# johannes-graeter/limo

Hardware: NVIDIA H100
Metric: BA windows/s (30 KF, 3k LM, 40k obs) (higher is better)
Workload: dtype f64

## Files before the change

limo_b200/csrc/kba_api.cu:

```cuda
#include <algorithm>
#include <atomic>
#include <chrono>
#include <cstdio>
#include <cstdlib>
#include <cstring>
#include <memory>
#include <string>
#include <thread>
#include <vector>

#include <cuda_runtime.h>

#include "kba_b200.h"
#include "kba_kernels.h"

using namespace kba;

static thread_local std::string g_last_error;
static thread_local bool g_force_host_pack = false;
static int fail(int code, const std::string& msg) {
    g_last_error = msg;
    return code;
}
#define CU(call)                                                                                              \
// ... 9 lines not shown
    bool own_stream = false;
    Counters counters;
    bool kernel_timing = false;
    cudaEvent_t ev0 = nullptr, ev1 = nullptr;
    std::vector<cudaEvent_t> ev_pool;
    int ev_used = 0;
    int sm_count = 132;
    cudaEvent_t ev_block = nullptr;
    bool blocking_sync = false;
    void* ws = nullptr;
    size_t ws_cap = 0;
};

static cudaError_t wait_event(kba_handle*, cudaEvent_t ev) { return cudaEventSynchronize(ev); }
static cudaError_t wait_stream(kba_handle* h) {
    if (!h->blocking_sync) return cudaStreamSynchronize(h->stream);
    if (!h->ev_block) {
        const cudaError_t e = cudaEventCreateWithFlags(&h->ev_block, cudaEventBlockingSync | cudaEventDisableTiming);
        if (e != cudaSuccess) return e;
    }
    const cudaError_t e = cudaEventRecord(h->ev_block, h->stream);
    if (e != cudaSuccess) return e;
    return cudaEventSynchronize(h->ev_block);
}

template <typename T>
struct Staged {
    T* h = nullptr;
    T* d = nullptr;
    size_t n = 0;
    int alloc(size_t count, bool host_copy) {
        n = count;
        const size_t bytes = std::max<size_t>(count, 1) * sizeof(T);
        if (cudaMalloc(&d, bytes) != cudaSuccess) return 1;
        if (host_copy && cudaMallocHost(&h, bytes) != cudaSuccess) return 1;
        return 0;
    }
    void release() {
        if (d) cudaFree(d);
        if (h) cudaFreeHost(h);
        d = nullptr; h = nullptr;
    }
    cudaError_t upload(cudaStream_t s) { return cudaMemcpyAsync(d, h, std::max<size_t>(n, 1) * sizeof(T), cudaMemcpyHostToDevice, s); }
    cudaError_t download(cudaStream_t s) { return cudaMemcpyAsync(h, d, std::max<size_t>(n, 1) * sizeof(T), cudaMemcpyDeviceToHost, s); }
};

struct kba_batch {
    kba_handle* h = nullptr;
    BatchDev bd{};
    std::vector<WinDesc> desc_h;
    Staged<WinDesc> desc;
    Staged<double> pose0, plane0, cam, lm0, lm_weight;
    Staged<uint8_t> kf_fixed;
    Staged<int> lm_ptr, obs_kf, obs_cam, obs_lm, kf_ptr, pm_lm, pm_cam, chunk_lm0, chunk_lm1, chunk_k0, chunk_k1, lm_orig, obs_orig;
    Staged<int> grp_k0, grp_k1;
    bool device_pack = false;
    Staged<int> r_lm_ptr, r_obs_kf, r_obs_cam, r_gp_lm;
    Staged<float> r_obs_u, r_obs_v, r_obs_d;
    Staged<double> r_lm_pos, r_lm_weight;
    Staged<double> lm_user;
    Staged<uint8_t> rej_user;
    PackRaw raw;
    Staged<int> obs_rank;
    Staged<float> obs_u, obs_v, obs_d, pm_u, pm_v, pm_d;
    Staged<WinState> state;
    Staged<IterRecord> log;
    Staged<double> pose_out[2], lm_out[2], plane_out[2];
    Staged<int> gp_lm, gp_kf, gp_of_lm, gp_shared;
    Staged<double> gp_weight;
    Staged<uint8_t> lm_active;
    Staged<int> n_active;
    Staged<unsigned long long> jac_obs;
    std::vector<void*> scratch;
    LaunchCfg lc;
    size_t h2d_bytes = 0, d2h_bytes = 0;
    float last_solve_ms = 0.f;
    cudaEvent_t ev_a = nullptr, ev_b = nullptr, ev_poll = nullptr, ev_poll2 = nullptr;
    struct SolveGraph {
        cudaGraph_t graph = nullptr;
        cudaGraphExec_t exec = nullptr;
        std::vector<unsigned char> key;
        Counters per_pass;
        int mode = 0, passes_per_launch = 0;
        bool unusable = false;
        void destroy() {
            if (exec) cudaGraphExecDestroy(exec);
            if (graph) cudaGraphDestroy(graph);
            exec = nullptr; graph = nullptr; key.clear();
        }
    } sg;
    Staged<int> loop_pass;
    long long solves_done = 0;
    int p_split_cap = 0;

    template <typename T>
    int dev_alloc(T** p, size_t count) {
        void* q = nullptr;
        if (cudaMalloc(&q, std::max<size_t>(count, 1) * sizeof(T)) != cudaSuccess) return 1;
        scratch.push_back(q);
        *p = (T*)q;
        return 0;
    }
    void dev_free(void* q) {
        scratch.erase(std::remove(scratch.begin(), scratch.end(), q), scratch.end());
        cudaFree(q);
    }
    void release() {
        desc.release(); pose0.release(); plane0.release(); cam.release(); lm0.release(); lm_weight.release();
        kf_fixed.release(); lm_ptr.release(); obs_kf.release(); obs_cam.release(); obs_lm.release(); kf_ptr.release();
        pm_lm.release(); pm_cam.release(); chunk_lm0.release(); chunk_lm1.release(); chunk_k0.release(); chunk_k1.release();
        lm_orig.release(); obs_orig.release(); obs_rank.release(); obs_u.release(); obs_v.release();
        grp_k0.release(); grp_k1.release();
        r_lm_ptr.release(); r_obs_kf.release(); r_obs_cam.release(); r_gp_lm.release(); r_obs_u.release(); r_obs_v.release();
        r_obs_d.release(); r_lm_pos.release(); r_lm_weight.release(); lm_user.release(); rej_user.release();
        obs_d.release(); pm_u.release(); pm_v.release(); pm_d.release(); state.release(); log.release();
        pose_out[0].release(); pose_out[1].release(); lm_out[0].release(); lm_out[1].release(); lm_active.release();
        n_active.release(); jac_obs.release(); plane_out[0].release(); plane_out[1].release();
        gp_lm.release(); gp_kf.release(); gp_of_lm.release(); gp_weight.release(); gp_shared.release();
        for (void* p : scratch) cudaFree(p);
        scratch.clear();
        if (ev_a) cudaEventDestroy(ev_a);
        if (ev_b) cudaEventDestroy(ev_b);
        if (ev_poll) cudaEventDestroy(ev_poll);
        if (ev_poll2) cudaEventDestroy(ev_poll2);
        sg.destroy();
        loop_pass.release();
    }
};

struct MotionBufs {
    Staged<unsigned char> up;
    Staged<unsigned char> out;
    double* run_pw = nullptr, *trim_val = nullptr;
    unsigned char* run_active = nullptr, *run_rej = nullptr;
    IterRecord* log = nullptr;
    cudaEvent_t ev0 = nullptr, ev1 = nullptr;
    int frames_cap = 0, runs_cap = 0, meas_cap = 0;
    std::vector<unsigned> seen;
    unsigned stamp = 0;
    static size_t al(size_t b) { return (b + 15) & ~(size_t)15; }
    static size_t up_bytes(int frames, int runs, int meas) {
        return al(sizeof(FrameDesc) * (size_t)frames) + al(4 * ((size_t)runs + frames)) + 5 * al(4 * (size_t)meas);
    }
    static size_t out_bytes(int frames, int log_cap, int runs) {
        return al(sizeof(FrameRes) * (size_t)frames) + al(sizeof(IterRecord) * (size_t)frames * log_cap) + al((size_t)runs);
    }
    int alloc(int frames, int runs, int meas) {
        frames_cap = frames; runs_cap = runs; meas_cap = meas;
        int bad = up.alloc(up_bytes(frames, runs, meas), true) | out.alloc(out_bytes(frames, kIterLogCap, runs), true);
        bad |= cudaMalloc(&run_pw, sizeof(double) * 4 * (size_t)std::max(runs, 1)) != cudaSuccess;
        bad |= cudaMalloc(&trim_val, sizeof(double) * 2 * (size_t)std::max(runs, 1)) != cudaSuccess;
        bad |= cudaMalloc(&run_active, (size_t)std::max(runs, 1)) != cudaSuccess;
        bad |= cudaMalloc(&run_rej, (size_t)std::max(runs, 1)) != cudaSuccess;
        bad |= cudaMalloc(&log, sizeof(IterRecord) * kIterLogCap * (size_t)frames) != cudaSuccess;
        bad |= cudaEventCreate(&ev0) != cudaSuccess;
        bad |= cudaEventCreate(&ev1) != cudaSuccess;
        return bad;
    }
    ~MotionBufs() {
        up.release(); out.release();
        if (run_pw) cudaFree(run_pw);
        if (trim_val) cudaFree(trim_val);
        if (run_active) cudaFree(run_active);
        if (run_rej) cudaFree(run_rej);
        if (log) cudaFree(log);
        if (ev0) cudaEventDestroy(ev0);
        if (ev1) cudaEventDestroy(ev1);
    }
};

struct TrackSolver {
// ... 186 lines not shown
            const int k = b->obs_kf.h[(size_t)d.obs_off + o];
            k0 = std::min(k0, k); k1 = std::max(k1, k);
        }
        for (int j = j0; j < j1; ++j)
            if (gp_kf_of_lm[j] >= 0) { k0 = std::min(k0, gp_kf_of_lm[j]); k1 = std::max(k1, gp_kf_of_lm[j]); }
        b->grp_k0.h[d.grp_off + c] = k0;
        b->grp_k1.h[d.grp_off + c] = k1;
    }
}

static void fill_window_raw(kba_batch* b, int wi, const kba_window* w) {
    const WinDesc& d = b->desc_h[wi];
    memcpy(b->pose0.h + 7 * (size_t)d.kf_off, w->kf_pose, sizeof(double) * 7 * w->n_kf);
    memcpy(b->kf_fixed.h + d.kf_off, w->kf_fixed, w->n_kf);
    for (int k = 0; k < w->n_kf; ++k) {
        double* pl = b->plane0.h + 4 * (size_t)(d.kf_off + k);
        if (w->kf_plane) memcpy(pl, w->kf_plane + 4 * k, 4 * sizeof(double));
        else { pl[0] = 0; pl[1] = 0; pl[2] = 1; pl[3] = 0; }
    }
    for (int c = 0; c < w->n_cam; ++c) {
        double* o = b->cam.h + kCamStride * (size_t)(d.cam_off + c);
        quat_to_rot<double>(w->cam_pose + 7 * c, o);
        o[9] = w->cam_pose[7 * c + 4]; o[10] = w->cam_pose[7 * c + 5]; o[11] = w->cam_pose[7 * c + 6];
        o[12] = w->cam_intr[3 * c]; o[13] = w->cam_intr[3 * c + 1]; o[14] = w->cam_intr[3 * c + 2]; o[15] = 0;
    }
    const size_t nl = (size_t)w->n_lm, no = (size_t)w->n_obs;
    memcpy(b->r_lm_pos.h + 3 * (size_t)d.lm_off, w->lm_pos, 3 * nl * sizeof(double));
    memcpy(b->r_lm_weight.h + d.lm_off, w->lm_weight, nl * sizeof(double));
    int* lp = b->r_lm_ptr.h + d.lm_off + wi;
    if (nl) memcpy(lp, w->lm_obs_ptr, (nl + 1) * sizeof(int)); else lp[0] = 0;
    memcpy(b->r_obs_kf.h + d.obs_off, w->obs_kf, no * sizeof(int));
    if (w->obs_cam) memcpy(b->r_obs_cam.h + d.obs_off, w->obs_cam, no * sizeof(int));
    else memset(b->r_obs_cam.h + d.obs_off, 0, no * sizeof(int));
    memcpy(b->r_obs_u.h + d.obs_off, w->obs_u, no * sizeof(float));
    memcpy(b->r_obs_v.h + d.obs_off, w->obs_v, no * sizeof(float));
    memcpy(b->r_obs_d.h + d.obs_off, w->obs_d, no * sizeof(float));
    if (w->n_gp) {
        memcpy(b->r_gp_lm.h + d.gp_off, w->gp_lm, w->n_gp * sizeof(int));
        memcpy(b->gp_kf.h + d.gp_off, w->gp_kf, w->n_gp * sizeof(int));
        memcpy(b->gp_weight.h + d.gp_off, w->gp_weight, w->n_gp * sizeof(double));
    }
    int max_rank = 0;
    for (int j = 0; j < w->n_lm; ++j) {
        int rank = 0;
        for (int o = w->lm_obs_ptr[j] + 1; o < w->lm_obs_ptr[j + 1]; ++o) {
            rank = (w->obs_kf[o] == w->obs_kf[o - 1]) ? rank + 1 : 0;
            max_rank = std::max(max_rank, rank);
        }
    }
    b->desc_h[wi].max_rank = max_rank;
    b->desc.h[wi].max_rank = max_rank;
}

static int window_rows(const kba_window& w) {
    const bool planes = w.n_gp > 0 || w.plane_reg_weight > 0;
    int n_free = 0;
    for (int k = 0; k < w.n_kf; ++k) n_free += w.kf_fixed[k] ? 0 : 1;
    return (planes ? 10 : 6) * n_free + 1;
}

struct kba_shard_comm;
kba::Exchange kba_shard_exchange(kba_shard_comm* c);

static int solve_graph_mode() {
    static const int m = [] {
        const char* e = getenv("KBA_GRAPH");
        const int v = e ? atoi(e) : 2;
        return (v < 0 || v > 2) ? 2 : v;
    }();
    return m;
}

static bool shard_graph_enabled() {
    static const bool on = [] { const char* e = getenv("KBA_SHARD_GRAPH"); return e ? atoi(e) != 0 : true; }();
    return on;
}

template <typename T>
static void key_append(std::vector<unsigned char>& k, const T& v) {
    const unsigned char* p = reinterpret_cast<const unsigned char*>(&v);
    k.insert(k.end(), p, p + sizeof(T));
}

static bool build_solve_graph(kba_batch* b, const SolveParams& sp, const LaunchCfg& lc, int mode, int max_passes, int check_every,
                              const std::vector<unsigned char>& key) {
    kba_batch::SolveGraph& g = b->sg;
    g.destroy();
    cudaStream_t s = b->h->stream;
    Counters per{};
    cudaError_t e = cudaSuccess;
    bool capturing = false;
    int rc_pass = 0;
    if (mode == 2) {
        cudaGraphConditionalHandle handle = 0;
        cudaGraphNode_t node = nullptr;
        cudaGraphNodeParams np = {};
        e = cudaGraphCreate(&g.graph, 0);
        if (e == cudaSuccess) e = cudaGraphConditionalHandleCreate(&handle, g.graph, 1, cudaGraphCondAssignDefault);
        if (e == cudaSuccess) {
            np.type = cudaGraphNodeTypeConditional;
            np.conditional.handle = handle;
            np.conditional.type = cudaGraphCondTypeWhile;
            np.conditional.size = 1;
            e = cudaGraphAddNode(&node, g.graph, nullptr, 0, &np);
        }
        if (e == cudaSuccess) e = cudaStreamBeginCaptureToGraph(s, np.conditional.phGraph_out[0], nullptr, nullptr, 0, cudaStreamCaptureModeThreadLocal);
        if (e == cudaSuccess) {
            capturing = true;
            rc_pass = launch_pass(b->bd, sp, lc, &per, s);
            launch_loop_cond(b->bd, (unsigned long long)handle, b->loop_pass.d, max_passes, s);
            cudaGraph_t body = nullptr;
            e = cudaStreamEndCapture(s, &body);
            capturing = false;
        }
        g.passes_per_launch = 0;
    } else {
        e = cudaStreamBeginCapture(s, cudaStreamCaptureModeThreadLocal);
        if (e == cudaSuccess) {
            capturing = true;
            for (int i = 0; i < check_every && !rc_pass; ++i) rc_pass = launch_pass(b->bd, sp, lc, i == 0 ? &per : nullptr, s);
            launch_count_active(b->bd, s);
            b->n_active.download(s);
            e = cudaStreamEndCapture(s, &g.graph);
            capturing = false;
        }
        g.passes_per_launch = check_every;
    }
    if (capturing) { cudaGraph_t junk = nullptr; cudaStreamEndCapture(s, &junk); }
    if (e == cudaSuccess && rc_pass) e = cudaErrorUnknown;
    if (e == cudaSuccess) e = cudaGraphInstantiate(&g.exec, g.graph, 0);
    if (e != cudaSuccess) {
        if (getenv("KBA_GRAPH_VERBOSE")) fprintf(stderr, "kba: solve graph (mode %d) not available: %s -- stream launches\n", mode, cudaGetErrorString(e));
        g.destroy();
        g.unusable = true;
        cudaGetLastError();
        return false;
    }
    if (getenv("KBA_GRAPH_VERBOSE")) fprintf(stderr, "kba: solve graph built (mode %d, %lld launches per pass)\n", mode, per.launches_total);
    g.key = key;
    g.per_pass = per;
    g.mode = mode;
    return true;
}

static void add_pass_counters(Counters& c, const Counters& per, long long passes) {
    c.launches_total += per.launches_total * passes; c.launches_jacobian += per.launches_jacobian * passes;
    c.launches_prep += per.launches_prep * passes; c.launches_schur += per.launches_schur * passes;
    c.launches_solve += per.launches_solve * passes; c.launches_backsub += per.launches_backsub * passes;
    c.launches_cost += per.launches_cost * passes; c.launches_update += per.launches_update * passes;
    c.launches_trim += per.launches_trim * passes;
}

extern "C" {

int kba_version(void) { return KBA_VERSION_MAJOR * 100 + KBA_VERSION_MINOR; }
int kba_internal_stream(kba_handle* h, cudaStream_t* s, int* device) {
    if (!h) return fail(KBA_ERR_BAD_ARG, "null handle");
    *s = h->stream; *device = h->device;
    return KBA_OK;
}
int kba_internal_fail(int code, const char* msg) { return fail(code, msg ? msg : ""); }
int kba_internal_workspace(kba_handle* h, size_t bytes, void** out) {
    if (!h || !out) return fail(KBA_ERR_BAD_ARG, "null handle");
    if (bytes > h->ws_cap) {
        CU(cudaSetDevice(h->device));
        CU(cudaStreamSynchronize(h->stream));
        if (h->ws) cudaFree(h->ws);
        h->ws = nullptr; h->ws_cap = 0;
        const size_t cap = bytes + bytes / 4 + 4096;
        CU(cudaMalloc(&h->ws, cap));
        h->ws_cap = cap;
    }
    *out = h->ws;
    return KBA_OK;
}
const char* kba_last_error(void) { return g_last_error.c_str(); }

void kba_default_options(kba_options* o) {
    if (!o) return;
    memset(o, 0, sizeof *o);
    o->depth_thres = 0.16; o->reprojection_thres = 1.6;
    o->depth_quantile = 0.95; o->reprojection_quantile = 0.95; o->gp_quantile = 1.0; o->gp_huber = 0.1;
    o->num_trim_rounds = -1; o->trim_solver_iterations = 2; o->final_solver_iterations = 100;
    o->min_landmarks_for_trimming = 100; o->min_residual_groups = 30; o->num_rounds_option = 1;
    o->solver_time_sec = 20.0;
    o->function_tolerance = 1e-6; o->gradient_tolerance = 1e-10; o->parameter_tolerance = 1e-8;
    o->initial_trust_region_radius = 1e4; o->max_trust_region_radius = 1e16; o->min_trust_region_radius = 1e-32;
    o->min_relative_decrease = 1e-3; o->min_lm_diagonal = 1e-6; o->max_lm_diagonal = 1e32;
    o->max_consecutive_invalid_steps = 5; o->precision = 0;
}

int kba_create(kba_handle** out, int device) {
    if (!out) return fail(KBA_ERR_BAD_ARG, "null out pointer");
    int n = 0;
    if (cudaGetDeviceCount(&n) != cudaSuccess || n == 0)
        return fail(KBA_ERR_CUDA, "no CUDA device available: the kba_b200 library has no CPU fallback");
    if (device < 0 || device >= n) return fail(KBA_ERR_BAD_ARG, "device index out of range");
    CU(cudaSetDevice(device));
    cudaDeviceProp prop;
    CU(cudaGetDeviceProperties(&prop, device));
    if (prop.major != 9 || prop.minor != 0)
        return fail(KBA_ERR_CUDA, "kba_b200 kernels are built for sm_90a (H100) only, device " + std::to_string(device) +
                                      " is sm_" + std::to_string(prop.major) + std::to_string(prop.minor));
    kba_handle* h = new kba_handle();
    h->device = device;
    h->sm_count = prop.multiProcessorCount;
    { const char* e = std::getenv("KBA_BLOCKING_SYNC"); h->blocking_sync = e && std::atoi(e) != 0; }
    CU(cudaStreamCreateWithFlags(&h->stream, cudaStreamNonBlocking));
    h->own_stream = true;
    CU(cudaEventCreate(&h->ev0));
    CU(cudaEventCreate(&h->ev1));
    *out = h;
    return KBA_OK;
}

void kba_destroy(kba_handle* h) {
    if (!h) return;
    if (h->own_stream && h->stream) cudaStreamDestroy(h->stream);
    if (h->ev0) cudaEventDestroy(h->ev0);
    if (h->ev1) cudaEventDestroy(h->ev1);
    if (h->ev_block) cudaEventDestroy(h->ev_block);
// ... 31 lines not shown

static int syrk_split(int nr_cap_max, int n_windows, int sm_count) {
    const int nb = nr_cap_max / 64, pairs = nb * (nb + 1) / 2;
    return std::min(16, (6 * sm_count + n_windows * pairs - 1) / (n_windows * pairs));
}

static void solve_layout(BatchDev& bd, int nr_cap_max, int n_windows, int sm_count) {
    bd.solve_tiled = (nr_cap_max <= 192 && !bd.solve_row_major) ? 1 : 0;
    const int split_dflt = (!bd.solve_tiled && n_windows <= 16) ? std::max(1, std::min(32, sm_count / n_windows)) : 0;
    const char* e = std::getenv("KBA_SOLVE_SPLIT");
    bd.solve_split = bd.solve_tiled ? 0 : (e ? std::atoi(e) : split_dflt);
}

static int batch_create(kba_handle* h, int32_t n_windows, const kba_window* w, const int* rows_of, bool track_large, kba_batch** out) {
    if (!h || !w || !out || n_windows <= 0) return fail(KBA_ERR_BAD_ARG, "bad argument to kba_batch_create");
    CU(cudaSetDevice(h->device));
    std::string why;
    for (int i = 0; i < n_windows; ++i) {
        const int rc = validate_window(&w[i], why);
        if (rc != KBA_OK) return fail(rc, "window " + std::to_string(i) + ": " + why);
        if (w[i].n_kf < 3 && !w[i].landmarks_fixed)
            return fail(KBA_ERR_NOT_ENOUGH_KF, "window " + std::to_string(i) + ": fewer than 3 keyframes");
    }
    kba_batch* b = new kba_batch();
    b->h = h;
    BatchDev& bd = b->bd;
    bd.n_win = n_windows;
    b->desc_h.resize(n_windows);
    long long kf = 0, cam = 0, lm = 0, obs = 0, chunks = 0, soff = 0, gp = 0, groups = 0;
    int max_rows = 0, max_rows_free = 0, max_groups = 1;
    int nr_cap_max = 64;
    for (int i = 0; i < n_windows; ++i) {
        WinDesc& d = b->desc_h[i];
        memset(&d, 0, sizeof d);
        d.n_kf = w[i].n_kf; d.n_cam = w[i].n_cam; d.n_lm = w[i].n_lm; d.n_obs = w[i].n_obs; d.n_gp = w[i].n_gp;
        d.kf_off = (int)kf; d.cam_off = (int)cam; d.lm_off = (int)lm; d.obs_off = (int)obs; d.gp_off = (int)gp;
        d.chunk_off = (int)chunks; d.n_chunks = (w[i].n_lm + 31) / 32;
        d.grp_off = (int)groups; d.n_groups = (w[i].n_lm + 7) / 8;
        groups += d.n_groups; max_groups = std::max(max_groups, d.n_groups);
        max_rows_free = std::max(max_rows_free, window_rows(w[i]));
        d.scale_kf0 = w[i].scale_kf0; d.scale_kf1 = w[i].scale_kf1;
        d.scale_weight = w[i].scale_weight; d.scale_value = w[i].scale_value;
        const bool planes = w[i].n_gp > 0 || w[i].plane_reg_weight > 0;
        const int rows = rows_of ? rows_of[i] : (planes ? 10 : 6) * w[i].n_kf + 1;
        max_rows = std::max(max_rows, rows);
        d.nr_cap = ((rows + 63) / 64) * 64;
        d.plane_reg_weight = w[i].plane_reg_weight; d.plane_dist_fixed = w[i].plane_dist_fixed;
        d.s_off = soff;
        soff += (long long)d.nr_cap * d.nr_cap;
        nr_cap_max = std::max(nr_cap_max, d.nr_cap);
        kf += w[i].n_kf; cam += w[i].n_cam; lm += w[i].n_lm; obs += w[i].n_obs; chunks += d.n_chunks; gp += w[i].n_gp;
        bd.max_obs = std::max(bd.max_obs, w[i].n_obs); bd.max_lm = std::max(bd.max_lm, w[i].n_lm);
        bd.max_kf = std::max(bd.max_kf, w[i].n_kf); bd.max_gp = std::max(bd.max_gp, w[i].n_gp);
    }
    if (obs > 2000000000LL) { b->release(); delete b; return fail(KBA_ERR_CAPACITY, "batch exceeds 2^31 observations"); }
    if (nr_cap_max > 640) {
        b->release();
        delete b;
        return fail(KBA_ERR_CAPACITY, "reduced system larger than 640 rows (106 keyframes, or 63 with ground-plane blocks)");
    }
    bd.tot_kf = kf; bd.tot_cam = cam; bd.tot_lm = lm; bd.tot_obs = obs; bd.tot_chunks = (int)chunks; bd.tot_gp = gp;
    bd.tot_groups = (int)groups;
    bd.nr_cap_max = nr_cap_max;
    b->lc.nr_cap_max = nr_cap_max;
    b->lc.sm_count = h->sm_count;
    {
        int max_chunks = 1;
        for (auto& d : b->desc_h) max_chunks = std::max(max_chunks, d.n_chunks);
        int p = syrk_split(nr_cap_max, n_windows, h->sm_count);
        b->lc.small_syrk = (max_rows <= 184);
        if (b->lc.small_syrk) p = (h->sm_count + n_windows - 1) / n_windows;
        bd.p_split = std::max(1, std::min(p, max_chunks));
        const char* fe = std::getenv("KBA_FUSED");
        bd.fused = (b->lc.small_syrk && bd.max_kf <= kFusedMaxKf && !(fe && std::atoi(fe) == 0)) ? 1 : 0;
        if (const char* pe = std::getenv("KBA_P_SPLIT")) { if (std::atoi(pe) > 0) p = std::atoi(pe); }
        if (bd.fused) bd.p_split = std::max(1, std::min(p, max_groups));
        else if (std::getenv("KBA_P_SPLIT")) bd.p_split = std::max(1, std::min(p, max_chunks));
        b->lc.fused_slots = (max_rows_free <= 176) ? 6 : 7;
    }
    bd.cost_parts = std::max((bd.max_obs + 255) / 256, (bd.max_obs / 16 + bd.max_lm / 32 + 4 + 7) / 8);
    { const char* le = std::getenv("KBA_LINEARIZE"); b->lc.lin_fused = !(le && std::atoi(le) == 0); }
    { const char* le = std::getenv("KBA_LIN_GRID"); if (le) b->lc.lin_grid = std::max(-1, std::atoi(le)); }
    { const char* le = std::getenv("KBA_BS_GRID"); if (le) b->lc.bs_grid = std::max(-1, std::atoi(le)); }
    {
        auto knob = [](const char* name, int dflt) { const char* e = std::getenv(name); return e ? std::atoi(e) : dflt; };
        bd.eval_tiles_jac = std::max(1, knob("KBA_EVAL_TILES_JAC", 8));
        bd.eval_tiles_cost = std::max(1, knob("KBA_EVAL_TILES_COST", 8));
        bd.eval_min_blocks = knob("KBA_EVAL_MIN_BLOCKS", 2);
        bd.eval_cs = knob("KBA_EVAL_CS", 0);
        bd.solve_row_major = knob("KBA_SOLVE_ROW_MAJOR", 0);
        solve_layout(bd, nr_cap_max, n_windows, h->sm_count);
    }
    bd.bs_parts = (bd.max_lm + 15) / 16;
    {
        const char* pe = std::getenv("KBA_DEVICE_PACK");
        b->device_pack = (bd.fused || track_large) && !g_force_host_pack && bd.max_lm <= pack_max_landmarks() && !(pe && std::atoi(pe) == 0);
    }
    if (track_large) {
        int max_chunks = 1;
        for (auto& d : b->desc_h) max_chunks = std::max(max_chunks, d.n_chunks);
        int p = syrk_split(192, n_windows, h->sm_count);
        if (const char* pe = std::getenv("KBA_P_SPLIT")) { if (std::atoi(pe) > 0) p = std::atoi(pe); }
        bd.p_split = std::max(bd.p_split, std::max(1, std::min(p, max_chunks)));
        b->p_split_cap = bd.p_split;
    }
    const bool hp = !b->device_pack;
    int bad = 0;
    bad |= b->desc.alloc(n_windows, true);
    bad |= b->pose0.alloc(7 * kf, true); bad |= b->plane0.alloc(4 * kf, true); bad |= b->kf_fixed.alloc(kf, true);
    bad |= b->cam.alloc(kCamStride * cam, true);
    bad |= b->lm0.alloc(3 * lm, hp); bad |= b->lm_weight.alloc(lm, hp); bad |= b->lm_ptr.alloc(lm + n_windows, hp);
    bad |= b->obs_kf.alloc(obs, hp); bad |= b->obs_cam.alloc(obs, hp); bad |= b->obs_lm.alloc(obs, hp);
    bad |= b->obs_u.alloc(obs, hp); bad |= b->obs_v.alloc(obs, hp); bad |= b->obs_d.alloc(obs, hp);
    bad |= b->kf_ptr.alloc(kf + n_windows, hp); bad |= b->pm_lm.alloc(obs, hp); bad |= b->pm_cam.alloc(obs, hp);
    bad |= b->pm_u.alloc(obs, hp); bad |= b->pm_v.alloc(obs, hp); bad |= b->pm_d.alloc(obs, hp);
    bad |= b->chunk_lm0.alloc(chunks, hp); bad |= b->chunk_lm1.alloc(chunks, hp);
    bad |= b->chunk_k0.alloc(chunks, hp); bad |= b->chunk_k1.alloc(chunks, hp);
    bad |= b->lm_orig.alloc(lm, hp); bad |= b->obs_rank.alloc(obs, hp);
    if (hp) bad |= b->obs_orig.alloc(obs, true);
    bad |= b->grp_k0.alloc(groups, hp); bad |= b->grp_k1.alloc(groups, hp);
    if (b->device_pack) {
        bad |= b->r_lm_ptr.alloc(lm + n_windows, true); bad |= b->r_obs_kf.alloc(obs, true); bad |= b->r_obs_cam.alloc(obs, true);
        bad |= b->r_obs_u.alloc(obs, true); bad |= b->r_obs_v.alloc(obs, true); bad |= b->r_obs_d.alloc(obs, true);
        bad |= b->r_lm_pos.alloc(3 * lm, true); bad |= b->r_lm_weight.alloc(lm, true); bad |= b->r_gp_lm.alloc(gp, true);
        bad |= b->lm_user.alloc(3 * lm, true); bad |= b->rej_user.alloc(lm, true);
        bad |= b->dev_alloc(&b->raw.lm_inv, lm);
    }
    bad |= b->dev_alloc(&bd.grp_t0, groups); bad |= b->dev_alloc(&bd.grp_t1, groups); bad |= b->dev_alloc(&bd.grp_rs, groups);
    bad |= b->dev_alloc(&bd.grp_tiles, groups);
    bad |= b->dev_alloc(&bd.lin_tile, (size_t)(obs / 16) + (size_t)(lm / 32) + 4 * (size_t)n_windows + 4);
#ifdef KBA_PROF
    bad |= b->dev_alloc(&bd.prof, 16);
    if (!bad) cudaMemset(bd.prof, 0, 16 * sizeof(unsigned long long));
#endif
    bad |= b->dev_alloc(&bd.rt[0], (size_t)kPoseStride * kf); bad |= b->dev_alloc(&bd.rt[1], (size_t)kPoseStride * kf);
    {
        bd.panel_cap = 0;
        bd.vpanel = nullptr;
        bad |= b->dev_alloc(&bd.chunk_poff, chunks); bad |= b->dev_alloc(&bd.chunk_rs, chunks);
    }
    bad |= b->dev_alloc(&bd.chunk_t0, chunks); bad |= b->dev_alloc(&bd.chunk_t1, chunks); bad |= b->dev_alloc(&bd.obs_row, obs);
    bad |= b->state.alloc(n_windows, true); bad |= b->log.alloc((size_t)n_windows * kIterLogCap, true);
    for (int q = 0; q < 2; ++q) { bad |= b->pose_out[q].alloc(7 * kf, true); bad |= b->lm_out[q].alloc(3 * lm, hp); }
    bad |= b->lm_active.alloc(lm, hp); bad |= b->n_active.alloc(1, true); bad |= b->jac_obs.alloc(1, true);
    bad |= b->plane_out[0].alloc(4 * kf, true); bad |= b->plane_out[1].alloc(4 * kf, true);
    bad |= b->gp_lm.alloc(gp, hp); bad |= b->gp_kf.alloc(gp, true); bad |= b->gp_weight.alloc(gp, true); bad |= b->gp_of_lm.alloc(lm, hp); bad |= b->gp_shared.alloc(gp, hp);
    bad |= b->dev_alloc(&bd.gp_lin, 14 * gp); bad |= b->dev_alloc(&bd.vgp, 30 * gp);
    bad |= b->dev_alloc(&bd.gp_cost_x, n_windows); bad |= b->dev_alloc(&bd.gp_cost_c, n_windows);
    bad |= b->dev_alloc(&bd.off_pose, kf); bad |= b->dev_alloc(&bd.off_dir, kf); bad |= b->dev_alloc(&bd.off_dist, kf);
    bad |= b->dev_alloc(&bd.bkf, 27 * kf);
    bad |= b->dev_alloc(&bd.scale_f, (size_t)n_windows * nr_cap_max); bad |= b->dev_alloc(&bd.lambda_f, (size_t)n_windows * nr_cap_max);
    bad |= b->dev_alloc(&bd.grad_f, (size_t)n_windows * nr_cap_max); bad |= b->dev_alloc(&bd.delta_f, (size_t)n_windows * nr_cap_max);
    bad |= b->dev_alloc(&bd.lm_scale, 3 * lm); bad |= b->dev_alloc(&bd.lm_linv, 6 * lm); bad |= b->dev_alloc(&bd.lm_z, 3 * lm);
    bad |= b->dev_alloc(&bd.lm_g, 3 * lm); bad |= b->dev_alloc(&bd.lm_lambda, 3 * lm); bad |= b->dev_alloc(&bd.trim_val, 3 * lm);
    bad |= b->dev_alloc(&bd.trim_reject, lm);
    bad |= b->dev_alloc(&bd.res, 3 * obs); bad |= b->dev_alloc(&bd.jp, 18 * obs);
    if (!bd.fused) bad |= b->dev_alloc(&bd.jl, 9 * obs);
    else { bad |= b->dev_alloc(&bd.vobs, 18 * obs); bad |= b->dev_alloc(&bd.lm_run, lm); }
    bad |= b->dev_alloc(&bd.cost_part_x, (size_t)n_windows * bd.cost_parts); bad |= b->dev_alloc(&bd.cost_part_c, (size_t)n_windows * bd.cost_parts);
    bad |= b->dev_alloc(&bd.bs_part, (size_t)n_windows * bd.bs_parts * 4);
    bad |= b->dev_alloc(&bd.sred, (size_t)soff * bd.p_split); bad |= b->dev_alloc(&bd.amat, (size_t)soff);
    bad |= b->dev_alloc(&bd.chol_w, (size_t)n_windows * 32 * 32); bad |= b->dev_alloc(&bd.chol_invd, (size_t)n_windows * nr_cap_max);
    if (bad) {
        const std::string msg = std::string("device/pinned allocation failed: ") + cudaGetErrorString(cudaGetLastError());
        b->release(); delete b;
        return fail(KBA_ERR_CUDA, msg);
// ... 114 lines not shown
        for (int i = 0; i < n_windows; ++i) { b->desc_h[i].panel_off = (long long)i * b->bd.panel_cap; b->desc.h[i].panel_off = b->desc_h[i].panel_off; }
    }
    cudaStream_t s = b->h->stream;
    if (b->device_pack) {
        CU(b->desc.upload(s)); CU(b->pose0.upload(s)); CU(b->plane0.upload(s)); CU(b->kf_fixed.upload(s)); CU(b->cam.upload(s));
        CU(b->r_lm_pos.upload(s)); CU(b->r_lm_weight.upload(s)); CU(b->r_lm_ptr.upload(s));
        CU(b->r_obs_kf.upload(s)); CU(b->r_obs_cam.upload(s)); CU(b->r_obs_u.upload(s)); CU(b->r_obs_v.upload(s)); CU(b->r_obs_d.upload(s));
        CU(b->r_gp_lm.upload(s)); CU(b->gp_kf.upload(s)); CU(b->gp_weight.upload(s));
        launch_pack(b->bd, b->raw, s);
        CU(cudaGetLastError());
        const BatchDev& bd = b->bd;
        b->h2d_bytes = sizeof(WinDesc) * bd.n_win + (7 + 4) * 8 * bd.tot_kf + bd.tot_kf + kCamStride * 8 * bd.tot_cam +
                       (3 + 1) * 8 * bd.tot_lm + 4 * (bd.tot_lm + bd.n_win) + (2 * 4 + 3 * 4) * bd.tot_obs + (4 + 4 + 8) * bd.tot_gp;
        return KBA_OK;
    }
    CU(b->desc.upload(s)); CU(b->pose0.upload(s)); CU(b->plane0.upload(s)); CU(b->kf_fixed.upload(s)); CU(b->cam.upload(s));
    CU(b->lm0.upload(s)); CU(b->lm_weight.upload(s)); CU(b->lm_ptr.upload(s));
    CU(b->obs_kf.upload(s)); CU(b->obs_cam.upload(s)); CU(b->obs_lm.upload(s));
    CU(b->obs_u.upload(s)); CU(b->obs_v.upload(s)); CU(b->obs_d.upload(s));
    CU(b->kf_ptr.upload(s)); CU(b->pm_lm.upload(s)); CU(b->pm_cam.upload(s)); CU(b->pm_u.upload(s)); CU(b->pm_v.upload(s)); CU(b->pm_d.upload(s));
    CU(b->chunk_lm0.upload(s)); CU(b->chunk_lm1.upload(s)); CU(b->chunk_k0.upload(s)); CU(b->chunk_k1.upload(s));
    CU(b->grp_k0.upload(s)); CU(b->grp_k1.upload(s));
    CU(b->lm_orig.upload(s)); CU(b->obs_rank.upload(s));
    CU(b->gp_lm.upload(s)); CU(b->gp_kf.upload(s)); CU(b->gp_weight.upload(s)); CU(b->gp_of_lm.upload(s)); CU(b->gp_shared.upload(s));
    const BatchDev& bd = b->bd;
    b->h2d_bytes = sizeof(WinDesc) * bd.n_win + (7 + 4) * 8 * bd.tot_kf + bd.tot_kf + kCamStride * 8 * bd.tot_cam +
                   (3 + 1) * 8 * bd.tot_lm + 4 * (bd.tot_lm + bd.n_win) + (3 * 4 + 3 * 4) * bd.tot_obs +
                   4 * (bd.tot_kf + bd.n_win) + (2 * 4 + 3 * 4) * bd.tot_obs + 8 * bd.tot_chunks + 8 * bd.tot_groups;
    return KBA_OK;
}

static SolveParams make_params(const kba_options* o) {
    SolveParams sp;
    sp.gp_huber = o->gp_huber; sp.gp_quantile = o->gp_quantile;
    sp.depth_thres = o->depth_thres; sp.reprojection_thres = o->reprojection_thres;
    sp.depth_quantile = o->depth_quantile; sp.reprojection_quantile = o->reprojection_quantile;
    sp.function_tolerance = o->function_tolerance; sp.gradient_tolerance = o->gradient_tolerance;
    sp.parameter_tolerance = o->parameter_tolerance; sp.initial_radius = o->initial_trust_region_radius;
    sp.max_radius = o->max_trust_region_radius; sp.min_radius = o->min_trust_region_radius;
    sp.min_relative_decrease = o->min_relative_decrease; sp.min_lm_diagonal = o->min_lm_diagonal;
    sp.max_lm_diagonal = o->max_lm_diagonal; sp.trim_solver_iterations = o->trim_solver_iterations;
    sp.final_solver_iterations = o->final_solver_iterations; sp.min_residual_groups = o->min_residual_groups;
    sp.max_consecutive_invalid_steps = o->max_consecutive_invalid_steps;
    sp.max_solver_time = o->solver_time_sec;
    return sp;
}

int kba_batch_solve(kba_batch* b, const kba_options* opt) {
    if (!b || !opt) return fail(KBA_ERR_BAD_ARG, "bad argument to kba_batch_solve");
    if (opt->precision != 0 && opt->precision != 1) return fail(KBA_ERR_BAD_ARG, "kba_options.precision must be 0 (FP64) or 1 (FP32 linearisation)");
    if (opt->num_trim_rounds > 6 || (opt->num_trim_rounds < 0 && opt->num_rounds_option > 6))
        return fail(KBA_ERR_CAPACITY, "at most 6 trimming rounds (KBA_MAX_SOLVES = 8 inner solves incl. one retry and the final solve)");
    b->bd.precision = opt->precision;
    b->bd.lin1 = (b->bd.fused && b->lc.lin_fused && opt->precision == 0 && b->lc.max_rank == 0) ? 1 : 0;
    kba_handle* h = b->h;
    CU(cudaSetDevice(h->device));
    cudaStream_t s = h->stream;
    const SolveParams sp = make_params(opt);
    LaunchCfg lc = b->lc;
    lc.rounds_override = opt->num_trim_rounds;
    lc.min_landmarks_for_trimming = opt->min_landmarks_for_trimming;
    lc.num_rounds_option = opt->num_rounds_option;
    lc.time_jacobian = h->kernel_timing;
    if (h->kernel_timing && h->ev_pool.empty()) {
        h->ev_pool.resize(1024);
        for (auto& e : h->ev_pool) CU(cudaEventCreate(&e));
    }
    h->ev_used = 0;
    lc.ev_pool = h->ev_pool.data(); lc.ev_cap = (int)h->ev_pool.size(); lc.ev_used = &h->ev_used;
    CU(cudaMemsetAsync(b->bd.jac_obs, 0, sizeof(unsigned long long), s));
    CU(cudaMemsetAsync(b->bd.cost_part_x, 0, sizeof(double) * (size_t)b->bd.n_win * b->bd.cost_parts, s));
    CU(cudaMemsetAsync(b->bd.cost_part_c, 0, sizeof(double) * (size_t)b->bd.n_win * b->bd.cost_parts, s));
    CU(cudaEventRecord(b->ev_a, s));
    launch_reset(b->bd, lc, s);
    const int rounds_max = 7;
    const int max_passes = rounds_max * (3 * opt->trim_solver_iterations + 4) + opt->final_solver_iterations + 8;
    const auto t0 = std::chrono::steady_clock::now();
    int check_every = 4;
    bool timed_out = false, poll_pending = false;
    int gmode = solve_graph_mode();
    if (h->kernel_timing || launch_check_enabled() || s == nullptr || b->sg.unusable) gmode = 0;
    const bool lockstep = b->bd.sharded != 0;
    if (lockstep) gmode = (gmode && shard_graph_enabled() && b->solves_done > 0) ? 1 : 0;
    if (gmode) {
        std::vector<unsigned char> key;
        key.reserve(sizeof(BatchDev) + sizeof(SolveParams) + 64);
        key_append(key, b->bd); key_append(key, sp); key_append(key, gmode); key_append(key, max_passes); key_append(key, s);
        key_append(key, lc.nr_cap_max); key_append(key, lc.max_rank); key_append(key, (int)lc.small_syrk); key_append(key, (int)lc.lin_fused);
        key_append(key, lc.fused_slots); key_append(key, lc.xchg.user);
        key_append(key, lc.lin_grid); key_append(key, lc.bs_grid);
        if (!(b->sg.exec && b->sg.key == key) && !build_solve_graph(b, sp, lc, gmode, max_passes, check_every, key)) gmode = 0;
    }
    if (gmode == 2) {
        CU(cudaMemsetAsync(b->loop_pass.d, 0, sizeof(int), s));
        CU(cudaGraphLaunch(b->sg.exec, s));
        CU(b->loop_pass.download(s));
        CU(cudaEventRecord(b->ev_b, s));
        CU(b->jac_obs.download(s));
        CU(wait_stream(h));
        CU(cudaGetLastError());
        CU(cudaEventElapsedTime(&b->last_solve_ms, b->ev_a, b->ev_b));
        h->counters.jacobian_obs += (long long)b->jac_obs.h[0];
        add_pass_counters(h->counters, b->sg.per_pass, b->loop_pass.h[0]);
        h->counters.launches_total += b->loop_pass.h[0];
        b->solves_done++;
        return KBA_OK;
    }
    if (gmode == 1) {
        cudaEvent_t evs[2] = {b->ev_poll, b->ev_poll2};
        const int n_launch = (max_passes + check_every - 1) / check_every;
        int launched = 0;
        for (int g = 0; g < n_launch; ++g) {
            CU(cudaGraphLaunch(b->sg.exec, s));
            ++launched;
            CU(cudaEventRecord(evs[g & 1], s));
            if (lockstep) {
                CU(wait_event(h, evs[g & 1]));
                if (b->n_active.h[0] == 0) break;
            } else if (g >= 1) {
                CU(wait_event(h, evs[(g - 1) & 1]));
                if (b->n_active.h[0] == 0) break;
                if (opt->solver_time_sec > 0) {
                    const double el = std::chrono::duration<double>(std::chrono::steady_clock::now() - t0).count();
                    if (el > KBA_MAX_SOLVES * opt->solver_time_sec + 2.0) { timed_out = true; break; }
                }
            }
        }
        if (timed_out) g_last_error = "kba_batch_solve: host safety cap reached, unfinished windows carry KBA_ERR_TIMEOUT in kba_result.status";
        CU(cudaEventRecord(b->ev_b, s));
        CU(b->jac_obs.download(s));
        CU(wait_stream(h));
        CU(cudaGetLastError());
        CU(cudaEventElapsedTime(&b->last_solve_ms, b->ev_a, b->ev_b));
        h->counters.jacobian_obs += (long long)b->jac_obs.h[0];
        add_pass_counters(h->counters, b->sg.per_pass, (long long)launched * check_every);
        h->counters.launches_total += launched;
        b->solves_done++;
        return KBA_OK;
    }
    for (int pass = 0; pass < max_passes; ++pass) {
        if (launch_pass(b->bd, sp, lc, &h->counters, s)) {
            cudaEventRecord(b->ev_b, s);
            return KBA_ERR_NCCL;
        }
        if (pass < 2) {
            const cudaError_t le = cudaGetLastError();
            if (le != cudaSuccess) { cudaEventRecord(b->ev_b, s); cudaStreamSynchronize(s); return fail(KBA_ERR_CUDA, std::string("kernel launch failed in kba_batch_solve: ") + cudaGetErrorString(le)); }
        }
        if ((pass + 1) % check_every == 0 || pass + 1 == max_passes) {
            if (poll_pending) {
                CU(wait_event(h, b->ev_poll));
                poll_pending = false;
                if (b->n_active.h[0] == 0) break;
                if (opt->solver_time_sec > 0 && !b->bd.sharded) {
                    const double el = std::chrono::duration<double>(std::chrono::steady_clock::now() - t0).count();
                    if (el > KBA_MAX_SOLVES * opt->solver_time_sec + 2.0) { timed_out = true; break; }
                }
            }
            launch_count_active(b->bd, s);
            CU(b->n_active.download(s));
            CU(cudaEventRecord(b->ev_poll, s));
            poll_pending = true;
        }
    }
    if (timed_out) g_last_error = "kba_batch_solve: host safety cap reached, unfinished windows carry KBA_ERR_TIMEOUT in kba_result.status";
    CU(cudaEventRecord(b->ev_b, s));
    CU(b->jac_obs.download(s));
    CU(wait_stream(h));
    CU(cudaGetLastError());
    CU(cudaEventElapsedTime(&b->last_solve_ms, b->ev_a, b->ev_b));
    h->counters.jacobian_obs += (long long)b->jac_obs.h[0];
    for (int i = 0; i + 1 < h->ev_used; i += 2) {
        float ms = 0.f;
// ... 899 lines not shown
```

limo_b200/csrc/kba_device.cuh:

```cuda
#pragma once
#include <cstdint>
#include <cuda_runtime.h>

namespace kba {

constexpr int kMaxKf = 128;
constexpr int kMaxCam = 8;
constexpr int kPoseStride = 12;
constexpr int kCamStride = 16;
constexpr int kIterLogCap = 160;
constexpr int kFusedMaxKf = 32;

struct WinDesc {
    int n_kf, n_cam, n_lm, n_obs, n_gp;
    int kf_off, cam_off, lm_off, obs_off, gp_off;
    int chunk_off, n_chunks;
    int grp_off, n_groups;
    int scale_kf0, scale_kf1;
    double scale_weight, scale_value;
    double plane_reg_weight;
    int plane_dist_fixed, landmarks_fixed;
    int speed_kf;
    int idle;
    double speed_weight, speed_dt;
    double speed_v_before[3];
    double speed_T_origin_before[7];
    long long s_off;
    int nr_cap;
    int max_rank;
    long long panel_off;
};

enum Phase : int { PH_SOLVE_BEGIN = 0, PH_ITERATE = 1, PH_TRIM = 2, PH_DONE = 3 };

struct SolveSummary {
    double initial_cost, final_cost;
    int num_iterations, num_successful_steps, termination, num_landmarks, num_residual_blocks, pad;
};

struct IterRecord {
    double cost, cost_change, gradient_max_norm, step_norm, relative_decrease, radius;
    int iteration, solve_index, valid, successful;
};

struct WinState {
    int phase;
    int cur;
    int need_linearize;
    int iter0;
    int solve_index;
    int round;
    int rounds_total;
    int retried;
    int is_final;
    int max_iter;
    int iteration;
    int num_invalid;
    int last_successful;
    int n_f;
    int nr;
    int eval_failed;
    int solve_failed;
    int log_n;
    int n_solves;
    int n_lin_tiles;
    double radius, decrease_factor;
    double x_cost, x_norm, gmax;
    double f_model, f_step_sq, f_xnorm_sq, f_gmax;
    unsigned long long t_solve_start;
    SolveSummary solves[8];
};

struct BatchDev {
    int n_win;
    int max_obs, max_lm, max_kf, max_gp;
    long long tot_obs, tot_lm, tot_kf, tot_cam, tot_gp;
    WinDesc* desc;
    WinState* state;
    IterRecord* log;
    double* pose0;
    double* plane0;
    double* pose[2];
    double* rt[2];
    double* plane[2];
    uint8_t* kf_fixed;
    int* off_pose;
    int* off_dir;
    int* off_dist;
    double* bkf;
    double* scale_f;
    double* cam;
    double* lm0;
    double* lm[2];
    double* lm_weight;
// ... 355 lines not shown
```

limo_b200/csrc/kba_kernels.cu:

```cuda
#include "kba_device.cuh"
#include "kba_kernels.h"
#include "kba_regularisers.cuh"
#include "kba_controller.cuh"
#include "kba_prep.cuh"
#include "kba_linearize.cuh"

#include <cfloat>
#include <cstdio>
#include <cstdlib>
#include <cmath>
#include <type_traits>

namespace kba {

constexpr int kBeginThreads = 1024;
__global__ void __launch_bounds__(kBeginThreads) k_solve_begin(BatchDev bd, SolveParams sp) {
    const int w = blockIdx.x;
    WinState& st = bd.state[w];
    if (st.phase != PH_SOLVE_BEGIN) return;
    const WinDesc wd = bd.desc[w];
    __shared__ int s_has[kMaxKf];
    __shared__ int s_plane[kMaxKf];
    __shared__ int s_cnt[3];
    __shared__ int s_tile_chunk[513];
    for (int k = threadIdx.x; k < wd.n_kf; k += blockDim.x) { s_has[k] = 0; s_plane[k] = 0; }
    if (threadIdx.x < 3) s_cnt[threadIdx.x] = 0;
    __syncthreads();
    {
        int n_gp_act = 0;
        for (int gi = threadIdx.x; gi < wd.n_gp; gi += blockDim.x) {
            const size_t G = (size_t)wd.gp_off + gi;
            if (!bd.lm_active[wd.lm_off + bd.gp_lm[G]]) continue;
            s_has[bd.gp_kf[G]] = 1;
            s_plane[bd.gp_kf[G]] = 1;
            n_gp_act++;
        }
        atomicAdd(&s_cnt[2], n_gp_act);
    }
    const int* lm_ptr = bd.lm_ptr + wd.lm_off + w;
    int n_lm_in = 0, n_blocks = 0;
    for (int j = threadIdx.x; j < wd.n_lm; j += blockDim.x) {
        if (!bd.lm_active[wd.lm_off + j]) continue;
        const int o0 = lm_ptr[j], o1 = lm_ptr[j + 1];
        if (o1 > o0) n_lm_in++;
        for (int o = o0; o < o1; ++o) {
            s_has[bd.obs_kf[wd.obs_off + o]] = 1;
            n_blocks += (bd.obs_d[wd.obs_off + o] > 0.0f) ? 2 : 1;
        }
    }
    atomicAdd(&s_cnt[0], n_lm_in);
    atomicAdd(&s_cnt[1], n_blocks);
    if (bd.sharded)
        for (int k = threadIdx.x; k < wd.n_kf; k += blockDim.x) s_has[k] = 1;
    __syncthreads();
    if (threadIdx.x == 0) {
        if (wd.scale_weight > 0) { s_has[wd.scale_kf0] = 1; s_has[wd.scale_kf1] = 1; }
        if (wd.speed_weight > 0) s_has[wd.speed_kf] = 1;
        if (wd.landmarks_fixed) s_cnt[0] = 0;
        const bool chain = wd.plane_reg_weight > 0 && wd.n_kf > 1;
        int n = 0, n_reg = 0;
        for (int k = 0; k < wd.n_kf; ++k) {
            const bool fixed = bd.kf_fixed[wd.kf_off + k];
            const bool var = (s_has[k] || chain) && !fixed;
            bd.off_pose[wd.kf_off + k] = var ? n : -1;
            if (var) n += 6;
            const bool pl = (s_plane[k] || chain) && !fixed;
            bd.off_dir[wd.kf_off + k] = pl ? n : -1;
            if (pl) n += 3;
            const bool pd = pl && !wd.plane_dist_fixed;
            bd.off_dist[wd.kf_off + k] = pd ? n : -1;
            if (pd) n += 1;
        }
        if (chain) n_reg = 3 * (wd.n_kf - 1) + wd.n_kf;
        st.n_f = n;
        st.nr = (n + 1 + 7) & ~7;
        st.radius = sp.initial_radius;
        st.decrease_factor = 2.0;
        st.iteration = 0;
        st.num_invalid = 0;
        st.last_successful = 0;
        st.need_linearize = 1;
        st.iter0 = 1;
        st.eval_failed = 0;
        st.solve_failed = 0;
        st.max_iter = st.is_final ? sp.final_solver_iterations
                                  : (st.retried ? 3 * sp.trim_solver_iterations : sp.trim_solver_iterations);
        SolveSummary& s = st.solves[st.solve_index];
        s.initial_cost = s.final_cost = 0.0;
        s.num_iterations = 0; s.num_successful_steps = 0; s.termination = 1;
        s.num_landmarks = s_cnt[0];
        s.num_residual_blocks = s_cnt[1] + s_cnt[2] + n_reg + (wd.scale_weight > 0 ? 1 : 0) + (wd.speed_weight > 0 ? 1 : 0);
        st.t_solve_start = global_timer_ns();
        st.phase = PH_ITERATE;
    }
    __syncthreads();
    for (int o = threadIdx.x; o < wd.n_obs; o += blockDim.x) {
        const size_t oo = (size_t)wd.obs_off + o;
        const bool act = bd.lm_active[wd.lm_off + bd.obs_lm[oo]];
        bd.obs_row[oo] = act ? bd.off_pose[wd.kf_off + bd.obs_kf[oo]] : -1;
// ... 6 lines not shown
            if (od >= 0) { r0 = min(r0, od); r1 = max(r1, od + 3); }
            if (oz >= 0) { r0 = min(r0, oz); r1 = max(r1, oz + 1); }
        }
        bd.chunk_t0[wd.chunk_off + c] = (r1 < 0) ? 0 : r0 / 8;
        bd.chunk_t1[wd.chunk_off + c] = (r1 < 0) ? 0 : (r1 + 7) / 8;
    }
    if (bd.fused) {
        __syncthreads();
        for (int j = threadIdx.x; j < wd.n_lm; j += blockDim.x) {
            const int o0 = lm_ptr[j], o1 = lm_ptr[j + 1];
            int n_start = 0, n_valid = 0, bad = 0, a = 0, row_a = 0, prev = -2;
            for (int o = o0; o < o1; ++o) {
                const size_t oo = (size_t)wd.obs_off + o;
                const int r = bd.obs_row[oo];
                if (r >= 0) {
                    ++n_valid;
                    if (prev < 0) { if (n_start++ == 0) { a = o - o0; row_a = r; } }
                    else if (r != prev + 6) bad = 1;
                    if (bd.obs_rank[oo] != 0) bad = 1;
                }
                prev = r;
            }
            int4 run = make_int4(0, 0, 0, 0);
            if (n_valid > 0) run = (bad || n_start != 1) ? make_int4(0, -1, 0, 0) : make_int4(a, n_valid, row_a, 0);
            bd.lm_run[wd.lm_off + j] = run;
        }
    }
    if (bd.fused) build_lin_tiles(bd, wd, st, w, s_tile_chunk);
    if (bd.fused) {
        const int trhs = st.n_f >> 3;
        for (int c = threadIdx.x; c < wd.n_groups; c += blockDim.x) {
            int r0 = 1 << 30, r1 = -1;
            for (int k = bd.grp_k0[wd.grp_off + c]; k <= bd.grp_k1[wd.grp_off + c]; ++k) {
                const int off = bd.off_pose[wd.kf_off + k], od = bd.off_dir[wd.kf_off + k], oz = bd.off_dist[wd.kf_off + k];
                if (off >= 0) { r0 = min(r0, off); r1 = max(r1, off + 6); }
                if (od >= 0) { r0 = min(r0, od); r1 = max(r1, od + 3); }
                if (oz >= 0) { r0 = min(r0, oz); r1 = max(r1, oz + 1); }
            }
            const int t0 = (r1 < 0) ? 0 : (r0 / 16) * 2, t1 = (r1 < 0) ? 0 : ((r1 + 15) / 16) * 2;
            int rows = 0;
            if (t1 > t0) rows = 8 * (t1 - t0) + ((trhs >= t0 && trhs < t1) ? 0 : 8);
            int e0 = 0, e1 = 0;
            if (t1 > t0) {
                e0 = r0 / 8;
                e1 = (r1 + 7) / 8;
                if (trhs >= t0 && trhs < t1) e1 = max(e1, trhs + 1);
            }
            bd.grp_t0[wd.grp_off + c] = t0;
            bd.grp_t1[wd.grp_off + c] = t1;
            bd.grp_tiles[wd.grp_off + c] = t0 | t1 << 8 | e0 << 16 | e1 << 24;
            bd.grp_rs[wd.grp_off + c] = rows;
        }
    }
    if (!bd.fused) {
        __syncthreads();
        if (threadIdx.x == 0) {
            const int trhs = st.n_f >> 3;
            int poff = 0;
            for (int c = 0; c < wd.n_chunks; ++c) {
                const int t0 = bd.chunk_t0[wd.chunk_off + c], t1 = bd.chunk_t1[wd.chunk_off + c];
                int rs = 0;
                if (t1 > t0) {
                    const int rows = 8 * (t1 - t0) + ((trhs >= t0 && trhs < t1) ? 0 : 8);
                    rs = ((rows - 4 + 15) / 16) * 16 + 4;
                }
                bd.chunk_rs[wd.chunk_off + c] = rs;
                bd.chunk_poff[wd.chunk_off + c] = poff;
                poff += 96 * rs;
            }
        }
    }
}

__global__ void __launch_bounds__(256) k_panel_zero(BatchDev bd) {
    const int w = blockIdx.y;
    if (bd.fused || bd.state[w].phase != PH_SOLVE_BEGIN || bd.desc[w].landmarks_fixed) return;
    double2* p = reinterpret_cast<double2*>(bd.vpanel + bd.desc[w].panel_off);
    const long long n2 = bd.panel_cap / 2;
    for (long long i = (long long)blockIdx.x * blockDim.x + threadIdx.x; i < n2; i += (long long)gridDim.x * blockDim.x)
        p[i] = make_double2(0.0, 0.0);
}

template <bool kJac, int kMinBlocks, typename TLin, bool kJl = true, bool kCs = false>
__global__ void __launch_bounds__(256, kMinBlocks) k_eval_obs(BatchDev bd, SolveParams sp, int tiles) {
    const int w = blockIdx.y;
    WinState& st = bd.state[w];
    const WinDesc& wd = bd.desc[w];
    const int n_obs = wd.n_obs, obs_off = wd.obs_off, lm_off = wd.lm_off;
    if (st.phase != PH_ITERATE) return;
    if (kJac && !st.need_linearize) return;
    if (!kJac && st.solve_failed) return;
    __shared__ __align__(16) double s_pose[kMaxKf * kPoseStride];
    __shared__ __align__(16) double s_cam[kMaxCam * kCamStride];
    __shared__ __align__(8) uint64_t s_bar;
    __shared__ double s_red[8];
    __shared__ int s_cnt[8];
    constexpr bool kF32 = sizeof(TLin) == 4;
    __shared__ float s_pose_f[kF32 ? kMaxKf * kPoseStride : 1];
    __shared__ float s_cam_f[kF32 ? kMaxCam * kCamStride : 1];
    const int buf = kJac ? st.cur : 1 - st.cur;
    const double* __restrict__ lm_buf = bd.lm[buf];
    const int i0 = blockIdx.x * tiles * 256 + threadIdx.x;
    int idx_b = (i0 < n_obs) ? bd.obs_lm[(size_t)obs_off + i0] : -1;
    int idx_a = (tiles > 1 && i0 + 256 < n_obs) ? bd.obs_lm[(size_t)obs_off + i0 + 256] : -1;
    int L = -1, kfi = 0, cami = 0, row = -1;
    float u = 0.f, v = 0.f, d = 0.f;
    double p0 = 0, p1 = 0, p2 = 0, wgt = 0;
    unsigned char act = 0;
    if (idx_b >= 0) {
        const size_t o = (size_t)obs_off + i0;
        L = lm_off + idx_b;
        kfi = bd.obs_kf[o]; cami = bd.obs_cam[o];
        if (kJac) row = bd.obs_row[o];
        u = bd.obs_u[o]; v = bd.obs_v[o]; d = bd.obs_d[o];
        p0 = lm_buf[3 * (size_t)L]; p1 = lm_buf[3 * (size_t)L + 1]; p2 = lm_buf[3 * (size_t)L + 2];
        wgt = bd.lm_weight[L];
        act = bd.lm_active[L];
    }
    stage_window_bulk(wd, bd.rt[buf], bd.cam, s_pose, s_cam, &s_bar);
    if (kF32) {
        for (int i = threadIdx.x; i < wd.n_kf * kPoseStride; i += blockDim.x) s_pose_f[i] = (float)s_pose[i];
        for (int i = threadIdx.x; i < wd.n_cam * kCamStride; i += blockDim.x) s_cam_f[i] = (float)s_cam[i];
        __syncthreads();
    }
    double cost = 0.0;
    int done = 0;
#pragma unroll 1
    for (int t = 0; t < tiles; ++t) {
        const int i_n = i0 + (t + 1) * 256;
        int Ln = -1, kfn = 0, camn = 0, rown = -1;
        float un = 0.f, vn = 0.f, dn = 0.f;
        double q0 = 0, q1 = 0, q2 = 0, wn = 0;
        unsigned char actn = 0;
        if (idx_a >= 0) {
            const size_t o = (size_t)obs_off + i_n;
            Ln = lm_off + idx_a;
            kfn = bd.obs_kf[o]; camn = bd.obs_cam[o];
            if (kJac) rown = bd.obs_row[o];
            un = bd.obs_u[o]; vn = bd.obs_v[o]; dn = bd.obs_d[o];
            q0 = lm_buf[3 * (size_t)Ln]; q1 = lm_buf[3 * (size_t)Ln + 1]; q2 = lm_buf[3 * (size_t)Ln + 2];
            wn = bd.lm_weight[Ln];
            actn = bd.lm_active[Ln];
        }
        idx_a = (t + 2 < tiles && i_n + 256 < n_obs) ? bd.obs_lm[(size_t)obs_off + i_n + 256] : -1;
        if (L >= 0 && act) {
            const size_t o = (size_t)obs_off + i0 + t * 256;
            const int k = kfi, c = cami;
            const double p[3] = {p0, p1, p2};
            double hr = 0.0;
            bool ok;
            if (kJac && kF32) {
                double r[3], raw[2];
                ok = eval_observation<double, false>(
                    s_pose + kPoseStride * k, s_cam + kCamStride * c, p, (double)u, (double)v, (double)d, wgt,
                    sp.reprojection_thres * sp.reprojection_thres, sp.depth_thres * sp.depth_thres, r, nullptr, nullptr, hr,
                    raw);
                if (ok) {
                    const float pf[3] = {(float)p0, (float)p1, (float)p2};
                    float hrf;
                    float* resf = reinterpret_cast<float*>(bd.res) + o;
                    float* jpf = reinterpret_cast<float*>(bd.jp) + o;
                    float* jlf = reinterpret_cast<float*>(bd.jl) + o;
                    eval_observation_store<float, kJl, kCs>(
                        s_pose_f + kPoseStride * k, s_cam_f + kCamStride * c, pf, u, v, d, (float)wgt,
                        (float)(sp.reprojection_thres * sp.reprojection_thres), (float)(sp.depth_thres * sp.depth_thres),
                        resf, jpf, jlf, (size_t)bd.tot_obs, row >= 0 || !kJl, hrf);
                }
            } else if (kJac) {
                ok = eval_observation_store<double, kJl, kCs>(
                    s_pose + kPoseStride * k, s_cam + kCamStride * c, p, (double)u, (double)v, (double)d, wgt,
                    sp.reprojection_thres * sp.reprojection_thres, sp.depth_thres * sp.depth_thres, bd.res + o, bd.jp + o,
                    bd.jl + o, (size_t)bd.tot_obs, row >= 0 || !kJl, hr);
            } else {
                double r[3], raw[2];
                ok = eval_observation<double, false>(
                    s_pose + kPoseStride * k, s_cam + kCamStride * c, p, (double)u, (double)v, (double)d, wgt,
                    sp.reprojection_thres * sp.reprojection_thres, sp.depth_thres * sp.depth_thres, r, nullptr, nullptr,
                    hr, raw);
            }
            if (!ok) {
                st.eval_failed = 1;
            } else {
                cost += hr;
                ++done;
            }
        }
        L = Ln; kfi = kfn; cami = camn; row = rown; u = un; v = vn; d = dn; p0 = q0; p1 = q1; p2 = q2; wgt = wn; act = actn;
    }
    cost = warp_sum(cost);
    if (kJac) done = __reduce_add_sync(0xffffffffu, done);
    if ((threadIdx.x & 31) == 0) { s_red[threadIdx.x >> 5] = cost; s_cnt[threadIdx.x >> 5] = done; }
    __syncthreads();
    if (threadIdx.x < tiles) {
        double s = 0.0;
        if (threadIdx.x == 0)
            for (int q = 0; q < 8; ++q) s += s_red[q];
        const int slot = blockIdx.x * tiles + threadIdx.x;
        if (slot < bd.cost_parts) (kJac ? bd.cost_part_x : bd.cost_part_c)[(size_t)w * bd.cost_parts + slot] = s;
    }
    if (kJac && threadIdx.x == 0) {
        int cnt = 0;
        for (int q = 0; q < 8; ++q) cnt += s_cnt[q];
        if (cnt) atomicAdd(bd.jac_obs, (unsigned long long)cnt);
    }
}

template <bool kJac>
static void launch_eval_obs(const BatchDev& bd, const SolveParams& sp, cudaStream_t s) {
    const int tiles = kJac ? bd.eval_tiles_jac : bd.eval_tiles_cost;
    const dim3 g((bd.max_obs + 256 * tiles - 1) / (256 * tiles), bd.n_win);
    if (!kJac) { k_eval_obs<false, 4, double><<<g, 256, 0, s>>>(bd, sp, tiles); return; }
    const int mb = bd.eval_min_blocks;
    if (bd.precision == 1) {
        if (bd.fused) k_eval_obs<true, 2, float, false><<<g, 256, 0, s>>>(bd, sp, tiles);
        else k_eval_obs<true, 2, float, true><<<g, 256, 0, s>>>(bd, sp, tiles);
        LCHK("k_eval_obs");
    } else if (!bd.fused) {
        if (mb == 2) k_eval_obs<true, 2, double, true><<<g, 256, 0, s>>>(bd, sp, tiles);
        else if (mb == 3) k_eval_obs<true, 3, double, true><<<g, 256, 0, s>>>(bd, sp, tiles);
        else k_eval_obs<true, 4, double, true><<<g, 256, 0, s>>>(bd, sp, tiles);
        LCHK("k_eval_obs");
    } else if (bd.eval_cs) {
        if (mb == 2) k_eval_obs<true, 2, double, false, true><<<g, 256, 0, s>>>(bd, sp, tiles);
        else if (mb == 3) k_eval_obs<true, 3, double, false, true><<<g, 256, 0, s>>>(bd, sp, tiles);
        else k_eval_obs<true, 4, double, false, true><<<g, 256, 0, s>>>(bd, sp, tiles);
        LCHK("k_eval_obs");
    } else {
        if (mb == 2) k_eval_obs<true, 2, double, false><<<g, 256, 0, s>>>(bd, sp, tiles);
        else if (mb == 3) k_eval_obs<true, 3, double, false><<<g, 256, 0, s>>>(bd, sp, tiles);
        else k_eval_obs<true, 4, double, false><<<g, 256, 0, s>>>(bd, sp, tiles);
        LCHK("k_eval_obs");
    }
}

template <bool kJac>
__global__ void __launch_bounds__(256) k_gp_eval(BatchDev bd, SolveParams sp) {
    const int w = blockIdx.x;
    const WinState& st = bd.state[w];
    if (st.phase != PH_ITERATE) return;
    if (kJac && !st.need_linearize) return;
    if (!kJac && st.solve_failed) return;
    const WinDesc& wd = bd.desc[w];
    if (wd.n_gp == 0) return;
    __shared__ double s_red[8];
    const int buf = kJac ? st.cur : 1 - st.cur;
    const size_t TG = (size_t)bd.tot_gp;
    double cost = 0.0;
    for (int gi = threadIdx.x; gi < wd.n_gp; gi += blockDim.x) {
        const size_t G = (size_t)wd.gp_off + gi;
        const int L = wd.lm_off + bd.gp_lm[G];
        if (!bd.lm_active[L]) continue;
        const int k = bd.gp_kf[G];
        const double* ps = bd.pose[buf] + 7 * (size_t)(wd.kf_off + k);
        const double* pl = bd.plane[buf] + 4 * (size_t)(wd.kf_off + k);
        const double* p = bd.lm[buf] + 3 * (size_t)L;
        double R[9];
        quat_to_rot<double>(ps, R);
        const double a[3] = {R[0] * p[0] + R[1] * p[1] + R[2] * p[2], R[3] * p[0] + R[4] * p[1] + R[5] * p[2],
                             R[6] * p[0] + R[7] * p[1] + R[8] * p[2]};
        const double px[3] = {a[0] + ps[4], a[1] + ps[5], a[2] + ps[6]};
        const double n[3] = {pl[0], pl[1], pl[2]};
        const double r = n[0] * px[0] + n[1] * px[1] + n[2] * px[2] + pl[3];
        const double s = r * r, ah = sp.gp_huber, wt = bd.gp_weight[G];
        double rho, rho1;
        if (s > ah * ah) { const double q = sqrt(s); rho = 2.0 * ah * q - ah * ah; rho1 = fmax(DBL_MIN, ah / q); }
        else { rho = s; rho1 = 1.0; }
        cost += 0.5 * wt * rho;
        if (kJac) {
            const double sq = sqrt(wt * rho1);
            double* o = bd.gp_lin + G;
            o[0] = sq * r;
            o[1 * TG] = sq * -2.0 * (n[1] * a[2] - n[2] * a[1]);
            o[2 * TG] = sq * -2.0 * (n[2] * a[0] - n[0] * a[2]);
            o[3 * TG] = sq * -2.0 * (n[0] * a[1] - n[1] * a[0]);
            o[4 * TG] = sq * n[0]; o[5 * TG] = sq * n[1]; o[6 * TG] = sq * n[2];
            const double nn = n[0] * n[0] + n[1] * n[1] + n[2] * n[2], inv = 1.0 / sqrt(nn);
            const double npx = (n[0] * px[0] + n[1] * px[1] + n[2] * px[2]) / nn;
            o[7 * TG] = sq * (px[0] - n[0] * npx) * inv;
            o[8 * TG] = sq * (px[1] - n[1] * npx) * inv;
            o[9 * TG] = sq * (px[2] - n[2] * npx) * inv;
            o[10 * TG] = sq;
            o[11 * TG] = sq * (n[0] * R[0] + n[1] * R[3] + n[2] * R[6]);
            o[12 * TG] = sq * (n[0] * R[1] + n[1] * R[4] + n[2] * R[7]);
            o[13 * TG] = sq * (n[0] * R[2] + n[1] * R[5] + n[2] * R[8]);
        }
    }
    cost = warp_sum(cost);
    if ((threadIdx.x & 31) == 0) s_red[threadIdx.x >> 5] = cost;
    __syncthreads();
    if (threadIdx.x == 0) {
        double s = 0.0;
        for (int q = 0; q < 8; ++q) s += s_red[q];
        (kJac ? bd.gp_cost_x : bd.gp_cost_c)[w] = s;
    }
}
template __global__ void k_gp_eval<true>(BatchDev, SolveParams);
template __global__ void k_gp_eval<false>(BatchDev, SolveParams);

__global__ void __launch_bounds__(256, 2) k_pose_hessian(BatchDev bd, SolveParams sp) {
    const int w = blockIdx.y, k = blockIdx.x;
    const WinState& st = bd.state[w];
    if (st.phase != PH_ITERATE || !st.need_linearize) return;
    const WinDesc& wd = bd.desc[w];
    if (k >= wd.n_kf || bd.off_pose[wd.kf_off + k] < 0) return;
    __shared__ double s_pose[kPoseStride];
    __shared__ double s_cam[kMaxCam * kCamStride];
    __shared__ double s_red[8][27];
    __shared__ double s_acc[9][256];
    __shared__ long long s_ob;
    __shared__ int s_lm_off, s_e1;
    if (threadIdx.x == 0) {
        s_ob = wd.obs_off; s_lm_off = wd.lm_off; s_e1 = bd.kf_ptr[wd.kf_off + w + k + 1];
        const double* p = bd.pose[st.cur] + 7 * (size_t)(wd.kf_off + k);
        double R[9];
        quat_to_rot<double>(p, R);
        for (int i = 0; i < 9; ++i) s_pose[i] = R[i];
        s_pose[9] = p[4]; s_pose[10] = p[5]; s_pose[11] = p[6];
    }
    for (int i = threadIdx.x; i < wd.n_cam * kCamStride; i += blockDim.x) s_cam[i] = bd.cam[(size_t)wd.cam_off * kCamStride + i];
    __syncthreads();
    double acc[18];
#pragma unroll
    for (int q = 0; q < 18; ++q) acc[q] = 0.0;
#pragma unroll
    for (int q = 0; q < 9; ++q) s_acc[q][threadIdx.x] = 0.0;
    const int* kp = bd.kf_ptr + wd.kf_off + w;
    const int e0 = kp[k], e1 = kp[k + 1];
    const double* __restrict__ lm_buf = bd.lm[st.cur];
    const size_t ob = (size_t)wd.obs_off;
    int e = e0 + threadIdx.x;
    int idx_b = (e < e1) ? bd.pm_lm[ob + e] : -1;
    int idx_a = (e + (int)blockDim.x < e1) ? bd.pm_lm[ob + e + blockDim.x] : -1;
    int L = -1, cam = 0;
    float u = 0.f, v = 0.f, d = 0.f;
    double p0 = 0, p1 = 0, p2 = 0, wgt = 0;
    unsigned char act = 0;
    if (idx_b >= 0) {
        L = wd.lm_off + idx_b;
        cam = bd.pm_cam[ob + e]; u = bd.pm_u[ob + e]; v = bd.pm_v[ob + e]; d = bd.pm_d[ob + e];
        p0 = lm_buf[3 * (size_t)L]; p1 = lm_buf[3 * (size_t)L + 1]; p2 = lm_buf[3 * (size_t)L + 2];
        wgt = bd.lm_weight[L]; act = bd.lm_active[L];
    }
#pragma unroll 1
    for (; e < s_e1; e += blockDim.x) {
        asm volatile("" ::: "memory");
        const size_t obs0 = (size_t)s_ob;
        const int e_end = s_e1, lm0 = s_lm_off;
        const int en = e + blockDim.x;
        int Ln = -1, camn = 0;
        float un = 0.f, vn = 0.f, dn = 0.f;
        double q0 = 0, q1 = 0, q2 = 0, wn = 0;
        unsigned char actn = 0;
        if (idx_a >= 0) {
            Ln = lm0 + idx_a;
            camn = bd.pm_cam[obs0 + en]; un = bd.pm_u[obs0 + en]; vn = bd.pm_v[obs0 + en]; dn = bd.pm_d[obs0 + en];
            q0 = lm_buf[3 * (size_t)Ln]; q1 = lm_buf[3 * (size_t)Ln + 1]; q2 = lm_buf[3 * (size_t)Ln + 2];
            wn = bd.lm_weight[Ln]; actn = bd.lm_active[Ln];
        }
        idx_a = (en + (int)blockDim.x < e_end) ? bd.pm_lm[obs0 + en + blockDim.x] : -1;
        if (act) {
            const double p[3] = {p0, p1, p2};
            double r[3], m[9], a[3], raw[2], hr;
            if (eval_factored<double, true, false>(s_pose, s_cam + kCamStride * cam, p, (double)u, (double)v, (double)d,
                                                   wgt, sp.reprojection_thres * sp.reprojection_thres,
                                                   sp.depth_thres * sp.depth_thres, r, m, a, hr, raw)) {
                double mm[6], h[3];
                gram_factored(m, mm);
#pragma unroll
                for (int c = 0; c < 3; ++c) h[c] = m[c] * r[0] + m[3 + c] * r[1] + m[6 + c] * r[2];
#pragma unroll
                for (int i = 0; i < 3; ++i) {
                    const int i1 = (i + 1) % 3, i2 = (i + 2) % 3;
                    double pr[3];
#pragma unroll
                    for (int c = 0; c < 3; ++c) pr[c] = 2.0 * (a[i1] * mm[sym3(i2, c)] - a[i2] * mm[sym3(i1, c)]);
                    const int qd = 6 * i - i * (i - 1) / 2;
#pragma unroll
                    for (int j = i; j < 3; ++j) {
                        const int j1 = (j + 1) % 3, j2 = (j + 2) % 3;
                        acc[qd + j - i] += 2.0 * (a[j1] * pr[j2] - a[j2] * pr[j1]);
                    }
#pragma unroll
                    for (int c = 0; c < 3; ++c) acc[qd + 3 - i + c] += pr[c];
                    acc[15 + i] += 2.0 * (a[i1] * h[i2] - a[i2] * h[i1]);
                }
#pragma unroll
                for (int q = 0; q < 6; ++q) s_acc[q][threadIdx.x] += mm[q];
#pragma unroll
                for (int c = 0; c < 3; ++c) s_acc[6 + c][threadIdx.x] += h[c];
            }
        }
        L = Ln; cam = camn; u = un; v = vn; d = dn; p0 = q0; p1 = q1; p2 = q2; wgt = wn; act = actn;
    }
#pragma unroll
    for (int q = 0; q < 27; ++q) {
        const double t = q < 15 ? acc[q] : q < 21 ? s_acc[q - 15][threadIdx.x] : q < 24 ? acc[q - 6] : s_acc[q - 18][threadIdx.x];
        const double v = warp_sum(t);
        if ((threadIdx.x & 31) == 0) s_red[threadIdx.x >> 5][q] = v;
    }
    __syncthreads();
    if (threadIdx.x < 27) {
        double s = 0.0;
        for (int q = 0; q < 8; ++q) s += s_red[q][threadIdx.x];
        bd.bkf[(size_t)(wd.kf_off + k) * 27 + threadIdx.x] = s;
    }
}

constexpr int kLC = 32;
constexpr int kKC = 3 * kLC;

__device__ __forceinline__ int gp_row(const BatchDev& bd, const WinDesc& wd, int k, int r) {
    if (r < 6) { const int o = bd.off_pose[wd.kf_off + k]; return o < 0 ? -1 : o + r; }
    if (r < 9) { const int o = bd.off_dir[wd.kf_off + k]; return o < 0 ? -1 : o + r - 6; }
    return bd.off_dist[wd.kf_off + k];
}

__device__ __forceinline__ void dmma(double& c0, double& c1, double a, double b) {
    asm volatile("mma.sync.aligned.m8n8k4.row.col.f64.f64.f64.f64 {%0,%1}, {%2}, {%3}, {%0,%1};\n"
                 : "+d"(c0), "+d"(c1)
                 : "d"(a), "d"(b));
}

constexpr int kGS = 64 + 4;

__global__ void __launch_bounds__(256, 2) k_schur_syrk(BatchDev bd) {
    const int w = blockIdx.z;
    const WinState& st = bd.state[w];
    if (st.phase != PH_ITERATE || st.solve_failed) return;
    const WinDesc& wd = bd.desc[w];
    if (wd.landmarks_fixed) return;
    int bi = 0, rem = blockIdx.x;
    while (rem > bi) { rem -= bi + 1; ++bi; }
    const int bj = rem;
    const int nrows = st.n_f + 1;
    if (bi * 64 >= nrows) return;
    const bool diag = (bi == bj);
    extern __shared__ double smem[];
    double* pa = smem;
    double* pb = diag ? pa : smem + kKC * kGS;
    const int warp = threadIdx.x >> 5, lane = threadIdx.x & 31;
    double acc[8][2];
#pragma unroll
    for (int t = 0; t < 8; ++t) acc[t][0] = acc[t][1] = 0.0;
    const int trhs = st.n_f >> 3;
    const bool a_rhs = trhs >= 8 * bi && trhs < 8 * bi + 8, b_rhs = trhs >= 8 * bj && trhs < 8 * bj + 8;
    const double* pbase = bd.vpanel + wd.panel_off;
    for (int ch = blockIdx.y; ch < wd.n_chunks; ch += bd.p_split) {
        const int t0 = bd.chunk_t0[wd.chunk_off + ch], t1 = bd.chunk_t1[wd.chunk_off + ch];
        const int rs = bd.chunk_rs[wd.chunk_off + ch];
        if (rs == 0) continue;
        const bool a_hit = (8 * bi < t1 && 8 * bi + 8 > t0) || a_rhs, b_hit = (8 * bj < t1 && 8 * bj + 8 > t0) || b_rhs;
        if (!(a_hit && b_hit)) continue;
        const double* pan = pbase + bd.chunk_poff[wd.chunk_off + ch];
        const bool rhs_in = trhs >= t0 && trhs < t1;
        __syncthreads();
        for (int idx = threadIdx.x; idx < (diag ? 1 : 2) * kKC * 64; idx += blockDim.x) {
            const int which = idx / (kKC * 64), e = idx - which * (kKC * 64);
            const int c = e >> 6, r = e & 63;
            const int g = 64 * (which ? bj : bi) + r, tile = g >> 3;
            double v = 0.0;
            if (tile >= t0 && tile < t1) v = pan[(size_t)c * rs + g - 8 * t0];
            else if (tile == trhs && !rhs_in) v = pan[(size_t)c * rs + 8 * (t1 - t0) + (g & 7)];
            (which ? pb : pa)[c * kGS + r] = v;
        }
        __syncthreads();
        const double* acol = pa + (lane & 3) * kGS + 8 * warp + (lane >> 2);
        const double* bcol = pb + (lane & 3) * kGS + (lane >> 2);
#pragma unroll 4
        for (int kk = 0; kk < kKC; kk += 4) {
            const double a = acol[kk * kGS];
#pragma unroll
            for (int t = 0; t < 8; ++t) {
                if (diag && t > warp) continue;
                dmma(acc[t][0], acc[t][1], a, bcol[kk * kGS + 8 * t]);
            }
        }
    }
    double* out = bd.sred + wd.s_off * (size_t)bd.p_split + (size_t)blockIdx.y * wd.nr_cap * wd.nr_cap;
    const int row = bi * 64 + 8 * warp + (lane >> 2);
#pragma unroll
    for (int t = 0; t < 8; ++t) {
        if (diag && t > warp) continue;
        const int col = bj * 64 + 8 * t + 2 * (lane & 3);
        out[(size_t)row * wd.nr_cap + col] = acc[t][0];
        out[(size_t)row * wd.nr_cap + col + 1] = acc[t][1];
    }
}
// ... 151 lines not shown
    double c[3], rc[3], d[3];
    for (int i = 0; i < 3; ++i) c[i] = R0[i] * t0[0] + R0[3 + i] * t0[1] + R0[6 + i] * t0[2];
    for (int i = 0; i < 3; ++i) rc[i] = R1[3 * i] * c[0] + R1[3 * i + 1] * c[1] + R1[3 * i + 2] * c[2];
    for (int i = 0; i < 3; ++i) d[i] = t1[i] - rc[i];
    const double nrm = sqrt(d[0] * d[0] + d[1] * d[1] + d[2] * d[2]);
    r = nrm - s0;
    if (!j1) return;
    const double u[3] = {d[0] / nrm, d[1] / nrm, d[2] / nrm};
    j1[0] = 2.0 * (u[1] * rc[2] - u[2] * rc[1]);
    j1[1] = 2.0 * (u[2] * rc[0] - u[0] * rc[2]);
    j1[2] = 2.0 * (u[0] * rc[1] - u[1] * rc[0]);
    j1[3] = u[0]; j1[4] = u[1]; j1[5] = u[2];
    double ur[3];
    double tmp[3];
    for (int i = 0; i < 3; ++i) tmp[i] = R1[i] * u[0] + R1[3 + i] * u[1] + R1[6 + i] * u[2];
    for (int i = 0; i < 3; ++i) ur[i] = R0[3 * i] * tmp[0] + R0[3 * i + 1] * tmp[1] + R0[3 * i + 2] * tmp[2];
    j0[3] = -ur[0]; j0[4] = -ur[1]; j0[5] = -ur[2];
    j0[0] = -2.0 * (ur[1] * t0[2] - ur[2] * t0[1]);
    j0[1] = -2.0 * (ur[2] * t0[0] - ur[0] * t0[2]);
    j0[2] = -2.0 * (ur[0] * t0[1] - ur[1] * t0[0]);
}

struct RowMajorMat {
    double* p; int ld;
    __device__ __forceinline__ double& operator()(int r, int c) const { return p[(size_t)r * ld + c]; }
};
struct TiledMat {
    double* p;
    __device__ __forceinline__ double* tile(int I, int J) const { return p + (size_t)(I * (I + 1) / 2 + J) * 64; }
    __device__ __forceinline__ double& operator()(int r, int c) const {
        return tile(r >> 3, c >> 3)[((c & 4) << 3) + ((r & 7) << 2) + (c & 3)];
    }
};

__device__ inline bool warp_chol32(double* D, int PS, double* inv, int lane) {
    bool ok = true;
#pragma unroll 1
    for (int jb = 0; jb < 4; ++jb) {
        const int c0 = 8 * jb;
        double r[8];
#pragma unroll
        for (int c = 0; c < 8; ++c) r[c] = D[lane * PS + c0 + c];
#pragma unroll 2
        for (int q = 0; q < c0; ++q) {
            const double lq = D[lane * PS + q];
#pragma unroll
            for (int c = 0; c < 8; ++c) r[c] -= lq * D[(c0 + c) * PS + q];
        }
#pragma unroll
        for (int j = 0; j < 8; ++j) {
            const double djj = __shfl_sync(0xffffffffu, r[j], c0 + j);
            if (!(djj > 0.0) || !isfinite(djj)) ok = false;
            const double rs = rsqrt(djj);
            const double lij = (lane == c0 + j) ? djj * rs : r[j] * rs;
            r[j] = lij;
            if (lane == c0 + j) inv[c0 + j] = rs;
#pragma unroll
            for (int c = j + 1; c < 8; ++c) {
                const double lcj = __shfl_sync(0xffffffffu, lij, c0 + c);
                r[c] -= lij * lcj;
            }
        }
        __syncwarp();
#pragma unroll
        for (int c = 0; c < 8; ++c) D[lane * PS + c0 + c] = (c0 + c <= lane) ? r[c] : 0.0;
        __syncwarp();
    }
    return ok;
}

#ifdef KBA_PHASE_CLOCKS
#define PHASE_DECL long long clk_[12] = {0, 0, 0, 0, 0, 0, 0, 0, 0, 0, 0, 0}; long long last_ = clock64()
#define PHASE_MARK(i) do { if (tid == 0 && w == 0) { clk_[i] = clock64(); last_ = clk_[i]; } } while (0)
#define PHASE_ACC(i) do { if (tid == 0 && w == 0) { const long long t_ = clock64(); clk_[i] += t_ - last_; last_ = t_; } } while (0)
#define PHASE_PRINT do { if (tid == 0 && w == 0) printf("reduced_solve cycles: sred %lld blocks %lld scale %lld chol %lld (diag %lld panel %lld trail %lld) backsub %lld tail %lld\n", clk_[1] - clk_[0], clk_[2] - clk_[1], clk_[3] - clk_[2], clk_[4] - clk_[3], clk_[8], clk_[9], clk_[10], clk_[5] - clk_[4], clk_[6] - clk_[5]); } while (0)
#else
#define PHASE_DECL
#define PHASE_MARK(i)
#define PHASE_ACC(i)
#define PHASE_PRINT
#endif

__global__ void __launch_bounds__(256) k_sred_reduce(BatchDev bd, int mode) {
    const int w = blockIdx.y;
    const WinState& st = bd.state[w];
    if (st.phase != PH_ITERATE || st.solve_failed) return;
    const WinDesc& wd = bd.desc[w];
    if (wd.landmarks_fixed) return;
    const int ld = wd.nr_cap, n = st.n_f;
    const int idx = blockIdx.x * blockDim.x + threadIdx.x;
    const bool pack = mode == 0 && bd.solve_tiled;
    const int rows_t = (n + 8) & ~7;
    if (idx >= (pack ? rows_t : n + 1) * ld) return;
    const int r = idx / ld, c = idx - r * ld;
    if (pack) {
        if (c >= rows_t || (c >> 3) > (r >> 3)) return;
        if (c > r || r > n) {
            TiledMat{bd.amat + wd.s_off}(r, c) = -0.0;
            return;
        }
    } else if (c > r) return;
    double* sp0 = bd.sred + wd.s_off * (size_t)bd.p_split;
    const size_t pstride = (size_t)ld * ld;
    double s = 0.0;
    int used = bd.p_split;
    if (bd.fused) { int per; schur_split(wd.n_groups, bd.p_split, per, used); }
    if (mode == 2) s = sp0[idx];
    else
    for (int p0 = 0; p0 < used; p0 += 16) {
        double v[16];
#pragma unroll
        for (int q = 0; q < 16; ++q) v[q] = (p0 + q < used) ? sp0[(size_t)(p0 + q) * pstride + idx] : 0.0;
#pragma unroll
        for (int q = 0; q < 16; ++q) s += v[q];
    }
    if (mode != 2) sp0[idx] = s;
    if (mode != 1 && !bd.solve_tiled) bd.amat[wd.s_off + idx] = (r == n && c == n) ? 0.0 : -s;
    if (pack) TiledMat{bd.amat + wd.s_off}(r, c) = (r == n && c == n) ? -0.0 : -s;
}

template <bool kTiled>
__global__ void __launch_bounds__(512, 1) k_reduced_solve(BatchDev bd, SolveParams sp, int stage) {
    const int w = blockIdx.x;
    WinState& st = bd.state[w];
    if (st.phase != PH_ITERATE) return;
    const WinDesc& wd = bd.desc[w];
    const int tid = threadIdx.x, nth = blockDim.x;
    const int n = st.n_f, ld = wd.nr_cap;
    extern __shared__ __align__(16) double sm[];
    double* s_fdiag = sm;
    double* s_g = s_fdiag + ld;
    double* s_y = s_g + ld;
    double* s_lam = s_y + ld;
    double* s_invd = s_lam + ld;
    double* s_inv = s_invd + ld;
    double* s_D = s_inv + kNB;
    double* s_P = s_D + kNB * (kNB + 1);
    using Mat = typename std::conditional<kTiled, TiledMat, RowMajorMat>::type;
    Mat A;
    if constexpr (kTiled) A.p = s_P;
    else { A.p = bd.amat + wd.s_off; A.ld = ld; }
    __shared__ int s_fail;
    __shared__ double s_red[16][4];
    if (tid == 0) s_fail = 0;
    PHASE_DECL;
    PHASE_MARK(0);
    if (stage == 2) {
        if (st.solve_failed) return;
        for (int c = tid; c < n; c += nth) {
            s_g[c] = bd.grad_f[(size_t)w * bd.nr_cap_max + c];
            s_lam[c] = bd.lambda_f[(size_t)w * bd.nr_cap_max + c];
            s_invd[c] = bd.chol_invd[(size_t)w * bd.nr_cap_max + c];
        }
        __syncthreads();
    }
    if (stage != 2) {
    const bool eval_cost = bd.lin1 ? (st.need_linearize && st.iter0) : (st.need_linearize != 0);
    if (eval_cost && tid < 32) {
        double c = 0.0;
        for (int q = tid; q < bd.cost_parts; q += 32) c += bd.cost_part_x[(size_t)w * bd.cost_parts + q];
        c = warp_sum(c);
        if (tid == 0) st.x_cost = c;
    }
    __syncthreads();
    if (st.eval_failed) {
        if (tid == 0) st.solve_failed = 2;
        return;
    }
    if (st.solve_failed) return;

    for (int i = tid; i < ld; i += nth) { s_fdiag[i] = 0.0; s_g[i] = 0.0; }
    {
        const double* sp0 = bd.sred + wd.s_off * (size_t)bd.p_split;
        const size_t pstride = (size_t)ld * ld;
        const int np = 1;
        const int rows = kTiled ? ((n + 8) & ~7) : n + 1;
        bool done_by_reduce = !kTiled && (bd.p_split > 1 || bd.sharded) && !wd.landmarks_fixed;
        if (kTiled && bd.p_split > 1 && !bd.sharded && !wd.landmarks_fixed) {
            const int ntr = rows >> 3;
            const int n2 = ntr * (ntr + 1) / 2 * 32;
            const double2* src = reinterpret_cast<const double2*>(bd.amat + wd.s_off);
            double2* dst = reinterpret_cast<double2*>(s_P);
            for (int i0 = tid; i0 < n2; i0 += 4 * nth) {
                double2 v[4];
#pragma unroll
                for (int u = 0; u < 4; ++u) if (i0 + u * nth < n2) v[u] = src[i0 + u * nth];
#pragma unroll
                for (int u = 0; u < 4; ++u) if (i0 + u * nth < n2) dst[i0 + u * nth] = v[u];
            }
            done_by_reduce = true;
        }
        const int total = done_by_reduce ? 0 : rows * ld;
        for (int idx0 = tid; idx0 < total; idx0 += 8 * nth) {
            double v[8];
            int rr[8], cc[8];
#pragma unroll
            for (int u = 0; u < 8; ++u) {
                const int idx = idx0 + u * nth;
                const int r = idx / ld, c = idx - r * ld;
                const bool skip = idx >= total || (kTiled ? (c >= rows || (c >> 3) > (r >> 3)) : (c > r || c >= n + 1));
                rr[u] = skip ? -1 : r; cc[u] = c;
                double s = 0.0;
                if (!skip && !wd.landmarks_fixed && c <= r && r <= n && !(r == n && c == n))
                    for (int p = 0; p < np; ++p) s += sp0[p * pstride + (size_t)r * ld + c];
                v[u] = s;
// ... 518 lines not shown
    const int j = blockIdx.x * 16 + grp;
    __shared__ double s_red[16][4];
    double model = 0.0, step_sq = 0.0, xn_sq = 0.0, gmax = 0.0;
    const bool have = j < wd.n_lm;
    const int L = wd.lm_off + (have ? j : 0);
    const double* pc = bd.lm[st.cur] + 3 * (size_t)L;
    double* pn = bd.lm[1 - st.cur] + 3 * (size_t)L;
    const int* lm_ptr = bd.lm_ptr + wd.lm_off + w;
    const int o0 = have ? lm_ptr[j] : 0, o1 = have ? lm_ptr[j + 1] : 0;
    const bool in = have && bd.lm_active[L] && o1 > o0 && !wd.landmarks_fixed && !st.solve_failed;
    const size_t base = (size_t)wd.obs_off;
    const double* delta_f = bd.delta_f + (size_t)w * bd.nr_cap_max;
    double t[3] = {0, 0, 0};
    const int gl = (in && wd.n_gp > 0) ? bd.gp_of_lm[L] : -1;
    bool mine = false;
    if (in) {
        const double* pcol = nullptr;
        int prs = 0, prow0 = 0;
        {
            const int ch = wd.chunk_off + (j >> 5);
            prs = bd.chunk_rs[ch];
            prow0 = 8 * bd.chunk_t0[ch];
            pcol = bd.vpanel + wd.panel_off + bd.chunk_poff[ch] + (size_t)(3 * (j & 31)) * prs;
        }
        const int gk = (gl >= 0) ? bd.gp_kf[wd.gp_off + gl] : -1;
        for (int o = o0 + hl; o < o1; o += 16) {
            if (gk >= 0) mine |= (bd.obs_kf[base + o] == gk);
            const int off = bd.obs_row[base + o];
            if (off < 0) continue;
            if (bd.obs_rank[base + o] != 0) continue;
            const double* q = pcol + (off - prow0);
#pragma unroll
            for (int r = 0; r < 6; ++r) {
                const double d = delta_f[off + r];
                t[0] += q[r] * d; t[1] += q[prs + r] * d; t[2] += q[2 * prs + r] * d;
            }
        }
    }
    const unsigned any = __ballot_sync(0xffffffffu, mine) & (0xffffu << (threadIdx.x & 16));
    if (gl >= 0 && hl < 10 && !(any != 0u && hl < 6)) {
        const int row = gp_row(bd, wd, bd.gp_kf[wd.gp_off + gl], hl);
        if (row >= 0) {
            const double d = delta_f[row];
#pragma unroll
            for (int c = 0; c < 3; ++c) t[c] += bd.vgp[(size_t)(3 * hl + c) * bd.tot_gp + wd.gp_off + gl] * d;
        }
    }
#pragma unroll
    for (int c = 0; c < 3; ++c)
#pragma unroll
        for (int m = 8; m >= 1; m >>= 1) t[c] += __shfl_xor_sync(0xffffffffu, t[c], m);
    if (have && hl == 0) {
        if (!in) {
            pn[0] = pc[0]; pn[1] = pc[1]; pn[2] = pc[2];
        } else {
            const double* z = bd.lm_z + 3 * (size_t)L;
            const double* li = bd.lm_linv + 6 * (size_t)L;
            const double t0 = t[0] + z[0], t1 = t[1] + z[1], t2 = t[2] + z[2];
            const double d0 = -(li[0] * t0 + li[1] * t1 + li[3] * t2);
            const double d1 = -(li[2] * t1 + li[4] * t2);
            const double d2 = -(li[5] * t2);
            const double* g = bd.lm_g + 3 * (size_t)L;
            const double* lam = bd.lm_lambda + 3 * (size_t)L;
            pn[0] = pc[0] + d0; pn[1] = pc[1] + d1; pn[2] = pc[2] + d2;
            model = -(g[0] * d0 + g[1] * d1 + g[2] * d2) + lam[0] * d0 * d0 + lam[1] * d1 * d1 + lam[2] * d2 * d2;
            step_sq = d0 * d0 + d1 * d1 + d2 * d2;
            xn_sq = pc[0] * pc[0] + pc[1] * pc[1] + pc[2] * pc[2];
            gmax = fmax(fabs(g[0]), fmax(fabs(g[1]), fabs(g[2])));
            if (!isfinite(d0) || !isfinite(d1) || !isfinite(d2)) model = nan("");
        }
    }
    if (hl == 0) { s_red[grp][0] = model; s_red[grp][1] = step_sq; s_red[grp][2] = xn_sq; s_red[grp][3] = gmax; }
    __syncthreads();
    if (threadIdx.x == 0) {
        double a = 0, b = 0, c = 0, g = 0;
        for (int q = 0; q < 16; ++q) { a += s_red[q][0]; b += s_red[q][1]; c += s_red[q][2]; g = fmax(g, s_red[q][3]); }
        double* out = bd.bs_part + ((size_t)w * bd.bs_parts + blockIdx.x) * 4;
        out[0] = a; out[1] = b; out[2] = c; out[3] = g;
    }
}

template <bool kLoop>
__global__ void __launch_bounds__(256) k_backsub_v(BatchDev bd, int n_units) {
    const int w = blockIdx.y;
    const WinState& st = bd.state[w];
    if (st.phase != PH_ITERATE) return;
    const WinDesc& wd = bd.desc[w];
    __shared__ double s_red[16][4];
    const int hl = threadIdx.x & 15, grp = threadIdx.x >> 4;
    for (int unit = blockIdx.x; unit < n_units; unit += gridDim.x) {
    const int j = unit * 16 + grp;
    double model = 0.0, step_sq = 0.0, xn_sq = 0.0, gmax = 0.0;
    const bool have = j < wd.n_lm;
    const int L = wd.lm_off + (have ? j : 0);
    const double* pc = bd.lm[st.cur] + 3 * (size_t)L;
    double* pn = bd.lm[1 - st.cur] + 3 * (size_t)L;
    const int* lm_ptr = bd.lm_ptr + wd.lm_off + w;
    const int o0 = have ? lm_ptr[j] : 0, o1 = have ? lm_ptr[j + 1] : 0;
    const bool in = have && bd.lm_active[L] && o1 > o0 && !wd.landmarks_fixed && !st.solve_failed;
    const size_t base = (size_t)wd.obs_off;
    const double* delta_f = bd.delta_f + (size_t)w * bd.nr_cap_max;
    double t[3] = {0, 0, 0};
    if (in) {
        for (int o = o0 + hl; o < o1; o += 16) {
            const int off = bd.obs_row[base + o];
            if (off < 0) continue;
            double d[6];
#pragma unroll
            for (int r = 0; r < 6; ++r) d[r] = delta_f[off + r];
#pragma unroll
            for (int c = 0; c < 3; ++c) {
                const double2* v = reinterpret_cast<const double2*>(bd.vobs + vobs_index(base, o0, o1, o, c));
#pragma unroll
                for (int h = 0; h < 3; ++h) {
                    const double2 x = v[h];
                    t[c] += x.x * d[2 * h] + x.y * d[2 * h + 1];
                }
            }
        }
        const int gl = (wd.n_gp > 0) ? bd.gp_of_lm[L] : -1;
        if (gl >= 0 && hl < 10) {
            const int row = gp_row(bd, wd, bd.gp_kf[wd.gp_off + gl], hl);
            if (row >= 0) {
                const double d = delta_f[row];
#pragma unroll
                for (int c = 0; c < 3; ++c) t[c] += bd.vgp[(size_t)(3 * hl + c) * bd.tot_gp + wd.gp_off + gl] * d;
            }
        }
    }
#pragma unroll
    for (int c = 0; c < 3; ++c)
#pragma unroll
        for (int m = 8; m >= 1; m >>= 1) t[c] += __shfl_xor_sync(0xffffffffu, t[c], m);
    if (have && hl == 0) {
        if (!in) {
            pn[0] = pc[0]; pn[1] = pc[1]; pn[2] = pc[2];
        } else {
            const double* z = bd.lm_z + 3 * (size_t)L;
            const double* li = bd.lm_linv + 6 * (size_t)L;
            const double t0 = t[0] + z[0], t1 = t[1] + z[1], t2 = t[2] + z[2];
            const double d0 = -(li[0] * t0 + li[1] * t1 + li[3] * t2);
            const double d1 = -(li[2] * t1 + li[4] * t2);
            const double d2 = -(li[5] * t2);
            const double* g = bd.lm_g + 3 * (size_t)L;
            const double* lam = bd.lm_lambda + 3 * (size_t)L;
            pn[0] = pc[0] + d0; pn[1] = pc[1] + d1; pn[2] = pc[2] + d2;
            model = -(g[0] * d0 + g[1] * d1 + g[2] * d2) + lam[0] * d0 * d0 + lam[1] * d1 * d1 + lam[2] * d2 * d2;
            step_sq = d0 * d0 + d1 * d1 + d2 * d2;
            xn_sq = pc[0] * pc[0] + pc[1] * pc[1] + pc[2] * pc[2];
            gmax = fmax(fabs(g[0]), fmax(fabs(g[1]), fabs(g[2])));
            if (!isfinite(d0) || !isfinite(d1) || !isfinite(d2)) model = nan("");
        }
    }
    if (hl == 0) { s_red[grp][0] = model; s_red[grp][1] = step_sq; s_red[grp][2] = xn_sq; s_red[grp][3] = gmax; }
    __syncthreads();
    if (threadIdx.x == 0) {
        double a = 0, b = 0, c = 0, g = 0;
        for (int q = 0; q < 16; ++q) { a += s_red[q][0]; b += s_red[q][1]; c += s_red[q][2]; g = fmax(g, s_red[q][3]); }
        double* out = bd.bs_part + ((size_t)w * bd.bs_parts + unit) * 4;
        out[0] = a; out[1] = b; out[2] = c; out[3] = g;
    }
    if constexpr (!kLoop) break;
    if (unit + (int)gridDim.x < n_units) __syncthreads();
    }
}

__global__ void __launch_bounds__(256) k_shard_scalars(BatchDev bd) {
    const WinState& st = bd.state[0];
    const WinDesc& wd = bd.desc[0];
    __shared__ double s_red[8][5];
    double a = 0, b = 0, c = 0, cc = 0, g = 0;
    if (st.phase == PH_ITERATE) {
        for (int q = threadIdx.x; q < (wd.n_lm + 15) / 16; q += blockDim.x) {
            const double* p = bd.bs_part + (size_t)q * 4;
            a += p[0]; b += p[1]; c += p[2]; g = fmax(g, p[3]);
        }
        for (int q = threadIdx.x; q < bd.cost_parts; q += blockDim.x) cc += bd.cost_part_c[q];
    }
    a = warp_sum(a); b = warp_sum(b); c = warp_sum(c); cc = warp_sum(cc); g = warp_max(g);
    if ((threadIdx.x & 31) == 0) {
        double* r = s_red[threadIdx.x >> 5];
        r[0] = a; r[1] = b; r[2] = c; r[3] = cc; r[4] = g;
    }
    __syncthreads();
    if (threadIdx.x == 0) {
        double t[5] = {0, 0, 0, 0, 0};
        for (int q = 0; q < 8; ++q) { for (int e = 0; e < 4; ++e) t[e] += s_red[q][e]; t[4] = fmax(t[4], s_red[q][4]); }
        bd.xs[0] = t[0]; bd.xs[1] = t[1]; bd.xs[2] = t[2]; bd.xs[3] = t[3];
        bd.xs[4] = (st.phase == PH_ITERATE && st.eval_failed) ? 1.0 : 0.0;
        for (int r = 0; r < bd.shard_world; ++r) bd.xs[16 + r] = (r == bd.shard_rank) ? t[4] : 0.0;
    }
}
__global__ void __launch_bounds__(256) k_shard_pack(BatchDev bd) {
    const WinState& st = bd.state[0];
    const WinDesc& wd = bd.desc[0];
    const size_t n_s = (size_t)wd.nr_cap * wd.nr_cap, n_b = (size_t)wd.n_kf * 27, n_c = (size_t)bd.cost_parts;
    const size_t i = (size_t)blockIdx.x * blockDim.x + threadIdx.x;
    const bool on = st.phase == PH_ITERATE;
    if (i < n_s) bd.x_send[i] = on ? bd.sred[i] : 0.0;
    else if (i < n_s + n_b) bd.x_send[i] = on ? bd.bkf[i - n_s] : 0.0;
    else if (i < n_s + n_b + n_c) bd.x_send[i] = on ? bd.cost_part_x[i - n_s - n_b] : 0.0;
    else if (i == n_s + n_b + n_c) bd.x_send[i] = (on && st.eval_failed) ? 1.0 : 0.0;
    else if (i == n_s + n_b + n_c + 1) bd.x_send[i] = (on && st.solve_failed) ? 1.0 : 0.0;
}
__global__ void k_shard_flags(BatchDev bd) {
    WinState& st = bd.state[0];
    if (threadIdx.x != 0 || st.phase != PH_ITERATE) return;
    const WinDesc& wd = bd.desc[0];
    const double* f = bd.x_recv + (size_t)wd.nr_cap * wd.nr_cap + (size_t)wd.n_kf * 27 + bd.cost_parts;
    if (f[0] > 0.0) st.eval_failed = 1;
    if (f[1] > 0.0 && !st.solve_failed) st.solve_failed = 1;
}
__global__ void __launch_bounds__(256) k_shard_trim_scatter(BatchDev bd) {
    const WinState& st = bd.state[0];
    if (st.phase != PH_TRIM) return;
    const WinDesc& wd = bd.desc[0];
    const int j = blockIdx.x * blockDim.x + threadIdx.x;
    if (j >= wd.n_lm) return;
    const int gidx = bd.lm_begin + bd.lm_orig[j];
    for (int g = 0; g < 3; ++g) bd.trim_send[(size_t)g * bd.lm_total + gidx] = bd.trim_val[(size_t)g * bd.tot_lm + j] + 2.0;
}

__global__ void __launch_bounds__(128) k_lm_update(BatchDev bd, SolveParams sp) {
    const int w = (blockIdx.x * blockDim.x + threadIdx.x) >> 5, lane = threadIdx.x & 31;
    if (w >= bd.n_win) return;
    WinState& st = bd.state[w];
    if (st.phase != PH_ITERATE) return;
    const WinDesc& wd = bd.desc[w];
    double e_model = 0, e_step = 0, e_xn = 0, e_g = 0, cand_sum = 0;
    for (int q = lane; q < (wd.n_lm + 15) / 16; q += 32) {
        const double* p = bd.bs_part + ((size_t)w * bd.bs_parts + q) * 4;
        e_model += p[0]; e_step += p[1]; e_xn += p[2]; e_g = fmax(e_g, p[3]);
    }
    for (int q = lane; q < bd.cost_parts; q += 32) cand_sum += bd.cost_part_c[(size_t)w * bd.cost_parts + q];
    e_model = warp_sum(e_model); e_step = warp_sum(e_step); e_xn = warp_sum(e_xn); e_g = warp_max(e_g);
    cand_sum = warp_sum(cand_sum);
    if (lane != 0) return;
    if (bd.sharded) {
        e_model = bd.xs[0]; e_step = bd.xs[1]; e_xn = bd.xs[2]; cand_sum = bd.xs[3];
        e_g = 0.0;
        for (int r = 0; r < bd.shard_world; ++r) e_g = fmax(e_g, bd.xs[16 + r]);
        if (bd.xs[4] > 0.0) st.eval_failed = 1;
    }
    const double* P = bd.pose[1 - st.cur];
    const double* PL = bd.plane[1 - st.cur];
    const double* gp_cost = bd.gp_cost_c + w;
    lm_step(st, bd.log + (size_t)w * kIterLogCap, sp, !bd.sharded, bd.lin1 != 0, e_model, e_step, e_xn, e_g,
            [&wd, cand_sum, P, PL, gp_cost]() {
        double cand = cand_sum;
        if (wd.scale_weight > 0) {
            double r;
            scale_regulariser(P + 7 * (size_t)(wd.kf_off + wd.scale_kf1), P + 7 * (size_t)(wd.kf_off + wd.scale_kf0),
                              wd.scale_value, r, nullptr, nullptr);
            cand += 0.5 * wd.scale_weight * r * r;
        }
        if (wd.speed_weight > 0) {
            double r[3];
            speed_regulariser(P + 7 * (size_t)(wd.kf_off + wd.speed_kf), wd.speed_T_origin_before, wd.speed_v_before, wd.speed_dt, r,
                              nullptr);
            cand += 0.5 * wd.speed_weight * (r[0] * r[0] + r[1] * r[1] + r[2] * r[2]);
        }
        if (wd.n_gp > 0) cand += *gp_cost;
        if (wd.plane_reg_weight > 0 && wd.n_kf > 1) cand += plane_chain_cost(wd, P, PL);
        return cand;
    });
}

__global__ void __launch_bounds__(256) k_trim_eval(BatchDev bd, SolveParams sp) {
    const int w = blockIdx.y;
    const WinState& st = bd.state[w];
    if (st.phase != PH_TRIM) return;
    const WinDesc& wd = bd.desc[w];
    __shared__ double s_pose[kMaxKf * kPoseStride];
    __shared__ double s_cam[kMaxCam * kCamStride];
    stage_window(wd, bd.pose[st.cur], bd.cam, s_pose, s_cam);
    __syncthreads();
    const int lane = threadIdx.x & 31;
    for (int it = 0; it < 8; ++it) {
    const int j = (blockIdx.x * 8 + it) * 8 + (threadIdx.x >> 5);
    if (j >= wd.n_lm) continue;
    const int L = wd.lm_off + j;
    double m_d = -1.0, m_r = -1.0;
    if (bd.lm_active[L]) {
        const int* lm_ptr = bd.lm_ptr + wd.lm_off + w;
        const double* lm = bd.lm[st.cur] + 3 * (size_t)L;
        const double p[3] = {lm[0], lm[1], lm[2]};
        for (int o = lm_ptr[j] + lane; o < lm_ptr[j + 1]; o += 32) {
            const size_t oo = (size_t)wd.obs_off + o;
            double r[3], raw[2], hr;
            if (!eval_observation<double, false>(s_pose + kPoseStride * bd.obs_kf[oo], s_cam + kCamStride * bd.obs_cam[oo],
                                                 p, (double)bd.obs_u[oo], (double)bd.obs_v[oo], (double)bd.obs_d[oo],
                                                 bd.lm_weight[L], sp.reprojection_thres * sp.reprojection_thres,
                                                 sp.depth_thres * sp.depth_thres, r, nullptr, nullptr, hr, raw))
                continue;
            m_r = fmax(m_r, raw[0]);
            m_d = fmax(m_d, raw[1]);
        }
        m_r = warp_max(m_r);
        m_d = warp_max(m_d);
    }
    if (lane == 0) {
        bd.trim_val[0 * (size_t)bd.tot_lm + L] = m_d;
        bd.trim_val[1 * (size_t)bd.tot_lm + L] = m_r;
        double m_g = -1.0;
        const int gl = (wd.n_gp > 0 && bd.lm_active[L]) ? bd.gp_of_lm[L] : -1;
        if (gl >= 0) {
            const int k = bd.gp_kf[wd.gp_off + gl];
            const double* ps = s_pose + kPoseStride * k;
            const double* pl = bd.plane[st.cur] + 4 * (size_t)(wd.kf_off + k);
            const double* lm = bd.lm[st.cur] + 3 * (size_t)L;
            double px[3];
            for (int i = 0; i < 3; ++i) px[i] = ps[3 * i] * lm[0] + ps[3 * i + 1] * lm[1] + ps[3 * i + 2] * lm[2] + ps[9 + i];
            m_g = fabs(pl[0] * px[0] + pl[1] * px[1] + pl[2] * px[2] + pl[3]);
        }
        bd.trim_val[2 * (size_t)bd.tot_lm + L] = m_g;
    }
    }
}

__global__ void __launch_bounds__(512) k_trim_select(BatchDev bd, SolveParams sp) {
    const int w = blockIdx.x;
    WinState& st = bd.state[w];
    if (st.phase != PH_TRIM) return;
    const WinDesc& wd = bd.desc[w];
    __shared__ TrimSmem s_trim;
    const double quant[3] = {sp.depth_quantile, sp.reprojection_quantile, sp.gp_quantile};
    const bool sh = bd.sharded != 0;
    const int n_items = sh ? bd.lm_total : wd.n_lm;
    const int* orig = bd.lm_orig + wd.lm_off;
    auto oid = [&](int j) { return sh ? j : orig[j]; };
    uint8_t* rej = sh ? bd.reject_glob : bd.trim_reject + wd.lm_off;
    for (int j = threadIdx.x; j < n_items; j += blockDim.x) rej[j] = 0;
    for (int g = 0; g < 3; ++g) {
        const double* vbase = sh ? bd.trim_glob + g * (size_t)bd.lm_total : bd.trim_val + g * (size_t)bd.tot_lm + wd.lm_off;
        const double voff = sh ? 2.0 : 0.0;
        auto val = [&](int j) { return vbase[j] - voff; };
        trim_select_group(s_trim, n_items, quant[g], sp.min_residual_groups, val, oid, rej);
    }
    __syncthreads();
    for (int j = threadIdx.x; j < wd.n_lm; j += blockDim.x)
        if (rej[sh ? bd.lm_begin + orig[j] : j]) bd.lm_active[wd.lm_off + j] = 0;
    __syncthreads();
    if (threadIdx.x == 0) trim_advance(st);
}

__global__ void k_count_active(BatchDev bd) {
    const int w = blockIdx.x * blockDim.x + threadIdx.x;
    if (w >= bd.n_win) return;
    if (bd.state[w].phase != PH_DONE) atomicAdd(bd.n_active, 1);
}

__global__ void k_reset_state(BatchDev bd, int rounds_total_override, int min_landmarks_for_trimming, int num_rounds_option) {
    const int w = blockIdx.x;
    const WinDesc& wd = bd.desc[w];
    for (int i = threadIdx.x; i < wd.n_kf * 7; i += blockDim.x) {
        const double v = bd.pose0[(size_t)wd.kf_off * 7 + i];
        bd.pose[0][(size_t)wd.kf_off * 7 + i] = v;
        bd.pose[1][(size_t)wd.kf_off * 7 + i] = v;
    }
    for (int k = threadIdx.x; k < wd.n_kf; k += blockDim.x) {
        double rt12[kPoseStride];
        write_rt(rt12, bd.pose0 + 7 * (size_t)(wd.kf_off + k));
        for (int i = 0; i < kPoseStride; ++i) {
            bd.rt[0][kPoseStride * (size_t)(wd.kf_off + k) + i] = rt12[i];
            bd.rt[1][kPoseStride * (size_t)(wd.kf_off + k) + i] = rt12[i];
        }
    }
    for (int i = threadIdx.x; i < wd.n_kf * 4; i += blockDim.x) {
        const double v = bd.plane0[(size_t)wd.kf_off * 4 + i];
        bd.plane[0][(size_t)wd.kf_off * 4 + i] = v;
        bd.plane[1][(size_t)wd.kf_off * 4 + i] = v;
    }
    for (int i = threadIdx.x; i < wd.n_lm * 3; i += blockDim.x) {
        const double v = bd.lm0[(size_t)wd.lm_off * 3 + i];
        bd.lm[0][(size_t)wd.lm_off * 3 + i] = v;
        bd.lm[1][(size_t)wd.lm_off * 3 + i] = v;
    }
    for (int i = threadIdx.x; i < wd.n_lm; i += blockDim.x) bd.lm_active[wd.lm_off + i] = 1;
    if (threadIdx.x == 0) {
        WinState& st = bd.state[w];
        st.phase = wd.idle ? PH_DONE : PH_SOLVE_BEGIN;
        st.cur = 0;
        st.solve_index = 0; st.round = 0; st.retried = 0; st.log_n = 0; st.n_solves = 0;
        int rounds = rounds_total_override;
        if (rounds < 0) rounds = ((bd.sharded ? bd.lm_total : wd.n_lm) > min_landmarks_for_trimming) ? num_rounds_option : 0;
        if (rounds > 6) rounds = 6;
        st.rounds_total = rounds;
        st.is_final = (rounds == 0);
        st.eval_failed = 0; st.solve_failed = 0;
    }
}

int launch_check_enabled() {
    static const int on = [] { const char* e = getenv("KBA_LAUNCH_CHECK"); return (e && e[0] == '1') ? 1 : 0; }();
    return on;
}
static cudaError_t g_launch_check_first = cudaSuccess;
void launch_check_report(const char* kernel, cudaError_t e) {
    if (g_launch_check_first == cudaSuccess) fprintf(stderr, "[kba] launch of %s failed: %s\n", kernel, cudaGetErrorString(e));
    g_launch_check_first = e;
}
static inline size_t schur_smem() { return (size_t)2 * kKC * kGS * sizeof(double); }
static inline size_t schur_tma_smem() { return (size_t)2 * kStageDoubles * sizeof(double); }
static inline size_t solve_smem(int ld) { return ((size_t)5 * ld + kNB + kNB * (kNB + 1) + (size_t)(ld + 8) * kPanelStride) * sizeof(double); }
static inline size_t trail_smem(int ld) { return (size_t)(ld + 8) * kPanelStride * sizeof(double); }
static inline size_t solve_tiled_smem(int ld) {
    const int nt = ld / 8;
    return ((size_t)5 * ld + kNB + kNB * (kNB + 1) + (size_t)nt * (nt + 1) / 2 * 64) * sizeof(double);
}

cudaError_t configure_kernels(int nr_cap_max) {
    static int hi_tiled[64] = {0}, hi_rows[64] = {0};
    static bool fixed_done[64] = {false};
    int dev = 0;
    cudaError_t e = cudaGetDevice(&dev);
    if (e != cudaSuccess) return e;
    dev &= 63;
    if (!fixed_done[dev]) {
        e = cudaFuncSetAttribute(k_schur_syrk, cudaFuncAttributeMaxDynamicSharedMemorySize, (int)schur_smem());
        if (e != cudaSuccess) return e;
        e = cudaFuncSetAttribute(k_schur_syrk_tma, cudaFuncAttributeMaxDynamicSharedMemorySize, (int)schur_tma_smem());
        if (e != cudaSuccess) return e;
        e = cudaFuncSetAttribute(k_schur_fused<6>, cudaFuncAttributeMaxDynamicSharedMemorySize, (int)schur_fused_smem());
        if (e != cudaSuccess) return e;
        e = cudaFuncSetAttribute(k_schur_fused<7>, cudaFuncAttributeMaxDynamicSharedMemorySize, (int)schur_fused_smem());
        if (e != cudaSuccess) return e;
        fixed_done[dev] = true;
    }
    if (nr_cap_max <= 192 && nr_cap_max > hi_tiled[dev]) {
        e = cudaFuncSetAttribute(k_reduced_solve<true>, cudaFuncAttributeMaxDynamicSharedMemorySize,
                                 (int)solve_tiled_smem(nr_cap_max));
        if (e != cudaSuccess) return e;
        hi_tiled[dev] = nr_cap_max;
    }
    if (nr_cap_max > hi_rows[dev]) {
        e = cudaFuncSetAttribute(k_chol_trail, cudaFuncAttributeMaxDynamicSharedMemorySize, (int)trail_smem(nr_cap_max));
        if (e != cudaSuccess) return e;
        e = cudaFuncSetAttribute(k_reduced_solve<false>, cudaFuncAttributeMaxDynamicSharedMemorySize, (int)solve_smem(nr_cap_max));
        if (e != cudaSuccess) return e;
        hi_rows[dev] = nr_cap_max;
    }
    return cudaSuccess;
}

static int strided_grid(int cfg, int n_units, int num, int den, int n_win, int sm_count, int ctas_per_sm, int waves) {
    if (cfg == 0) return n_units;
    if (cfg > 0) return cfg < n_units ? cfg : n_units;
    const int g = (n_units * num + den - 1) / den;
    return ((long long)g * n_win >= (long long)waves * ctas_per_sm * sm_count && g >= 1) ? g : n_units;
}

void launch_reset(const BatchDev& bd, const LaunchCfg& lc, cudaStream_t s) {
    k_reset_state<<<bd.n_win, 256, 0, s>>>(bd, lc.rounds_override, lc.min_landmarks_for_trimming, lc.num_rounds_option); LCHK("k_reset_state");
}

int launch_pass(const BatchDev& bd, const SolveParams& sp, const LaunchCfg& lc, Counters* cnt, cudaStream_t s) {
    const int B = bd.n_win;
    const dim3 g_obs((bd.max_obs + 255) / 256, B);
    const dim3 g_lm((bd.max_lm + 63) / 64, B);
    if (!bd.fused) k_panel_zero<<<dim3(64, B), 256, 0, s>>>(bd);
    LCHK("k_panel_zero");
    k_solve_begin<<<B, kBeginThreads, 0, s>>>(bd, sp); LCHK("k_solve_begin");
    const bool timed = lc.time_jacobian && lc.ev_pool && *lc.ev_used + 2 <= lc.ev_cap;
    const bool lin1 = bd.lin1 != 0;
    if (lin1) {
        if (bd.tot_gp > 0) k_gp_eval<true><<<B, 256, 0, s>>>(bd, sp);
        LCHK("k_gp_eval");
        if (timed) cudaEventRecord(lc.ev_pool[(*lc.ev_used)++], s);
        const int n_units = (lin_tile_bound(bd.max_obs, bd.max_lm) + kLinWarps - 1) / kLinWarps;
        const dim3 g_lin(strided_grid(lc.lin_grid, n_units, 1, 8, B, lc.sm_count, kLinMinBlocks, 6), B);
        if ((int)g_lin.x < n_units) k_linearize<true><<<g_lin, kLinThreads, 0, s>>>(bd, sp, n_units);
        else k_linearize<false><<<g_lin, kLinThreads, 0, s>>>(bd, sp, n_units);
        LCHK("k_linearize");
        if (timed) cudaEventRecord(lc.ev_pool[(*lc.ev_used)++], s);
        k_pose_hessian<<<dim3(bd.max_kf, B), 256, 0, s>>>(bd, sp); LCHK("k_pose_hessian");
    } else {
        if (timed) cudaEventRecord(lc.ev_pool[(*lc.ev_used)++], s);
        launch_eval_obs<true>(bd, sp, s);
        if (timed) cudaEventRecord(lc.ev_pool[(*lc.ev_used)++], s);
        if (bd.tot_gp > 0) k_gp_eval<true><<<B, 256, 0, s>>>(bd, sp);
        LCHK("k_gp_eval");
        k_pose_hessian<<<dim3(bd.max_kf, B), 256, 0, s>>>(bd, sp); LCHK("k_pose_hessian");
    }
    if (bd.fused) {
        if (!lin1) {
            k_landmark_reduce<true><<<dim3((bd.max_lm + 15) / 16, B), 256, 0, s>>>(bd, sp); LCHK("k_landmark_reduce");
            k_obs_v2<<<g_obs, 256, 0, s>>>(bd); LCHK("k_obs_v2");
        }
        const dim3 gf(bd.p_split, B);
        if (lc.fused_slots == 7) k_schur_fused<7><<<gf, 512, schur_fused_smem(), s>>>(bd);
        else k_schur_fused<6><<<gf, 512, schur_fused_smem(), s>>>(bd);
        LCHK("k_schur_fused");
    } else {
        k_landmark_reduce<false><<<dim3((bd.max_lm + 15) / 16, B), 256, 0, s>>>(bd, sp); LCHK("k_landmark_reduce");
        for (int round = 0; round <= lc.max_rank; ++round) k_obs_v<<<g_obs, 256, 0, s>>>(bd, round);
        LCHK("k_obs_v");
        if (bd.tot_gp > 0) k_gp_panel<<<dim3((bd.max_gp * 10 + 255) / 256, B), 256, 0, s>>>(bd);
        LCHK("k_gp_panel");
    }
    if (bd.fused) {
    } else if (lc.small_syrk) {
        k_schur_syrk_tma<<<dim3(bd.p_split, B), 512, schur_tma_smem(), s>>>(bd); LCHK("k_schur_syrk_tma");
    } else {
        const int nb = lc.nr_cap_max / 64;
        k_schur_syrk<<<dim3(nb * (nb + 1) / 2, bd.p_split, B), 256, schur_smem(), s>>>(bd); LCHK("k_schur_syrk");
    }
    const dim3 g_red((lc.nr_cap_max * lc.nr_cap_max + 255) / 256, B);
    BatchDev bc = bd;
    if (bd.sharded) {
        if (bd.p_split > 1) k_sred_reduce<<<g_red, 256, 0, s>>>(bd, 1);
        LCHK("k_sred_reduce");
        const LaunchCfg::WinDescHost& wh = lc.shard_win;
        const long long n_s = (long long)wh.nr_cap * wh.nr_cap, n_b = (long long)wh.n_kf * 27, n_x = n_s + n_b + bd.cost_parts + 2;
        k_shard_pack<<<(unsigned)((n_x + 255) / 256), 256, 0, s>>>(bd); LCHK("k_shard_pack");
        if (int rc = lc.xchg.allreduce(lc.xchg.user, bd.x_send, bd.x_recv, n_x, 0, s)) return rc;
        k_shard_flags<<<1, 32, 0, s>>>(bd); LCHK("k_shard_flags");
        bc.sred = bd.x_recv; bc.bkf = bd.x_recv + n_s; bc.cost_part_x = bd.x_recv + n_s + n_b;
        k_sred_reduce<<<g_red, 256, 0, s>>>(bc, 2); LCHK("k_sred_reduce");
    } else if (bd.p_split > 1) {
        k_sred_reduce<<<g_red, 256, 0, s>>>(bd, 0); LCHK("k_sred_reduce");
    }
    if (bd.solve_tiled) {
        k_reduced_solve<true><<<B, 512, solve_tiled_smem(lc.nr_cap_max), s>>>(bc, sp, 0); LCHK("k_reduced_solve");
    } else if (!bd.solve_split) {
        k_reduced_solve<false><<<B, 512, solve_smem(lc.nr_cap_max), s>>>(bc, sp, 0); LCHK("k_reduced_solve");
    } else {
        k_reduced_solve<false><<<B, 512, solve_smem(lc.nr_cap_max), s>>>(bc, sp, 1); LCHK("k_reduced_solve");
        const int strips = (lc.nr_cap_max + 7) / 8;
        for (int kb = 0; kb < lc.nr_cap_max; kb += kNB) {
            k_chol_diag<<<B, 32, 0, s>>>(bc, kb); LCHK("k_chol_diag");
            k_chol_panel<<<dim3((strips + 15) / 16, B), 512, 0, s>>>(bc, kb); LCHK("k_chol_panel");
            k_chol_trail<<<dim3(bd.solve_split, B), 512, trail_smem(lc.nr_cap_max), s>>>(bc, kb); LCHK("k_chol_trail");
        }
        k_reduced_solve<false><<<B, 512, solve_smem(lc.nr_cap_max), s>>>(bc, sp, 2); LCHK("k_reduced_solve");
    }
    if (bd.fused) {
        const int n_units = (bd.max_lm + 15) / 16;
        const int gx = strided_grid(lc.bs_grid, n_units, 1, 3, B, lc.sm_count, 2, 8);
        if (gx < n_units) k_backsub_v<true><<<dim3(gx, B), 256, 0, s>>>(bd, n_units);
        else k_backsub_v<false><<<dim3(n_units, B), 256, 0, s>>>(bd, n_units);
    }
    else k_backsub<<<dim3((bd.max_lm + 15) / 16, B), 256, 0, s>>>(bd);
    LCHK("k_backsub");
    launch_eval_obs<false>(bd, sp, s);
    if (bd.tot_gp > 0) k_gp_eval<false><<<B, 256, 0, s>>>(bd, sp);
    LCHK("k_gp_eval");
    if (bd.sharded) {
        k_shard_scalars<<<1, 256, 0, s>>>(bd); LCHK("k_shard_scalars");
        if (int rc = lc.xchg.allreduce(lc.xchg.user, bd.xs, bd.xs, 16 + bd.shard_world, 0, s)) return rc;
    }
    k_lm_update<<<(B * 32 + 127) / 128, 128, 0, s>>>(bd, sp); LCHK("k_lm_update");
    k_trim_eval<<<g_lm, 256, 0, s>>>(bd, sp); LCHK("k_trim_eval");
    if (bd.sharded) {
        k_shard_trim_scatter<<<(bd.max_lm + 255) / 256, 256, 0, s>>>(bd); LCHK("k_shard_trim_scatter");
        if (int rc = lc.xchg.allreduce(lc.xchg.user, bd.trim_send, bd.trim_glob, 3LL * bd.lm_total, 0, s)) return rc;
    }
    k_trim_select<<<B, 512, 0, s>>>(bd, sp); LCHK("k_trim_select");
    if (cnt) {
        const int gp = bd.tot_gp > 0 ? 1 : 0;
        const int prep = lin1 ? 1 : 2 + (bd.fused ? 1 : lc.max_rank + 1 + gp);
        const int split = (!bd.solve_tiled && bd.solve_split) ? 1 + 3 * ((lc.nr_cap_max + kNB - 1) / kNB) : 0;
        cnt->launches_total += (bd.fused ? 0 : 1) + 1 + 1 + gp + prep + 1 + (bd.p_split > 1 ? 1 : 0) + 1 + split + 1 + 1 + gp + 1 + 2;
        cnt->launches_jacobian += 1; cnt->launches_prep += prep + gp; cnt->launches_schur += 1; cnt->launches_solve += 2;
        cnt->launches_backsub += 1; cnt->launches_cost += 1 + gp; cnt->launches_update += 1; cnt->launches_trim += 2;
    }
    return 0;
}

void launch_count_active(const BatchDev& bd, cudaStream_t s) {
    cudaMemsetAsync(bd.n_active, 0, sizeof(int), s);
    k_count_active<<<(bd.n_win + 127) / 128, 128, 0, s>>>(bd); LCHK("k_count_active");
}

__global__ void __launch_bounds__(256) k_loop_cond(BatchDev bd, cudaGraphConditionalHandle handle, int* pass, int max_passes) {
    int active = 0;
    for (int w = threadIdx.x; w < bd.n_win; w += blockDim.x) active += (bd.state[w].phase != PH_DONE) ? 1 : 0;
    active = __syncthreads_count(active > 0);
    if (threadIdx.x == 0) {
        const int p = *pass + 1;
        *pass = p;
        *bd.n_active = active;
        cudaGraphSetConditional(handle, (active > 0 && p < max_passes) ? 1u : 0u);
    }
}
void launch_loop_cond(const BatchDev& bd, unsigned long long handle, int* pass, int max_passes, cudaStream_t s) {
    k_loop_cond<<<1, 256, 0, s>>>(bd, (cudaGraphConditionalHandle)handle, pass, max_passes);
}

__global__ void k_force_linearize(BatchDev bd) {
    const int w = blockIdx.x * blockDim.x + threadIdx.x;
    if (w >= bd.n_win) return;
    WinState& st = bd.state[w];
    st.phase = PH_ITERATE; st.need_linearize = 1; st.iter0 = 1; st.cur = 0; st.eval_failed = 0; st.solve_failed = 0;
}
void launch_jacobian_only(const BatchDev& bd, const SolveParams& sp, cudaStream_t s) {
    const dim3 g_obs((bd.max_obs + 255) / 256, bd.n_win);
    launch_eval_obs<true>(bd, sp, s);
}
template <typename TLin>
__global__ void k_expand_jl(BatchDev bd, TLin* out) {
    const WinDesc& wd = bd.desc[0];
    const int i = blockIdx.x * blockDim.x + threadIdx.x;
    if (i >= wd.n_obs) return;
    const size_t o = (size_t)wd.obs_off + i, T = (size_t)bd.tot_obs;
    const double* R = bd.rt[0] + kPoseStride * (size_t)(wd.kf_off + bd.obs_kf[o]);
    const TLin* jp = reinterpret_cast<const TLin*>(bd.jp);
    for (int r = 0; r < 3; ++r) {
        const double m0 = (double)jp[(6 * r + 3) * T + o], m1 = (double)jp[(6 * r + 4) * T + o], m2 = (double)jp[(6 * r + 5) * T + o];
        for (int c = 0; c < 3; ++c) out[(size_t)(3 * r + c) * T + o] = (TLin)(m0 * R[c] + m1 * R[3 + c] + m2 * R[6 + c]);
    }
}
void launch_expand_jl(const BatchDev& bd, double* out, cudaStream_t s) {
    const int n = (int)bd.tot_obs;
    if (bd.precision) k_expand_jl<float><<<(n + 255) / 256, 256, 0, s>>>(bd, reinterpret_cast<float*>(out));
    else k_expand_jl<double><<<(n + 255) / 256, 256, 0, s>>>(bd, out);
    LCHK("k_expand_jl");
}
void launch_force_linearize(const BatchDev& bd, cudaStream_t s) {
    k_solve_begin<<<bd.n_win, kBeginThreads, 0, s>>>(bd, SolveParams{}); LCHK("k_solve_begin");
    k_force_linearize<<<(bd.n_win + 127) / 128, 128, 0, s>>>(bd); LCHK("k_force_linearize");
}

}
```

limo_b200/csrc/kba_kernels.h:

```cpp
#pragma once
#include <cuda_runtime.h>

#include "kba_device.cuh"

namespace kba {

int launch_check_enabled();
void launch_check_report(const char* kernel, cudaError_t e);
#define LCHK(name)                                                                       \
    do {                                                                                 \
        if (kba::launch_check_enabled()) {                                               \
            const cudaError_t lchk_e_ = cudaGetLastError();                              \
            if (lchk_e_ != cudaSuccess) kba::launch_check_report(name, lchk_e_);         \
        }                                                                                \
    } while (0)

struct Counters {
    long long launches_total = 0;
    long long launches_jacobian = 0, launches_prep = 0, launches_schur = 0, launches_solve = 0, launches_backsub = 0,
              launches_cost = 0, launches_update = 0, launches_trim = 0;
    double ms_jacobian = 0.0;
    long long jacobian_obs = 0;
};

struct Exchange {
    int (*allreduce)(void* user, const double* send, double* recv, long long count, int op, cudaStream_t s) = nullptr;
    void* user = nullptr;
    int rank = 0, world = 1;
};

struct LaunchCfg {
    int nr_cap_max = 64;
    int sm_count = 132;
    int max_rank = 0;
    bool small_syrk = false;
    bool lin_fused = true;
    int lin_grid = -1;
    int bs_grid = -1;
    int fused_slots = 6;
    int rounds_override = -1, min_landmarks_for_trimming = 100, num_rounds_option = 1;
    bool time_jacobian = false;
    cudaEvent_t* ev_pool = nullptr;
    int ev_cap = 0;
    int* ev_used = nullptr;
    Exchange xchg;
    struct WinDescHost { int nr_cap = 0, n_kf = 0; } shard_win;
};

struct PackRaw {
    const int* lm_ptr = nullptr;
    const int* obs_kf = nullptr;
    const int* obs_cam = nullptr;
    const float* obs_u = nullptr, *obs_v = nullptr, *obs_d = nullptr;
    const double* lm_pos = nullptr;
    const double* lm_weight = nullptr;
    const int* gp_lm = nullptr;
    int* lm_inv = nullptr;
    int* obs_orig = nullptr;
};
struct TrackDev {
    double* kf_pose = nullptr;
    double* kf_plane = nullptr;
    int* m_off = nullptr;
    int* m_cnt = nullptr;
    int* m_lm = nullptr;
    int* m_cam = nullptr;
    float* m_u = nullptr, *m_v = nullptr, *m_d = nullptr;
    double* lm_pos = nullptr;
    double* lm_weight = nullptr;
    int* sel_index = nullptr;
    int* cursor = nullptr;
    long long* key = nullptr;
    int* n_depth = nullptr;
    int kf_cap = 0, lm_cap = 0, m_cap = 0;
};
struct TrackSel {
    const int* kf_slot = nullptr;
    const unsigned char* kf_fixed = nullptr;
    const int* lm_slot = nullptr;
    int n_kf = 0, n_lm = 0, max_meas = 0;
    int auto_scale = 0;
    const int* gp_cand = nullptr;
    int n_cand = 0;
};
struct TrackGrid {
    int max_kf = 0, max_lm = 0, max_meas = 0;
    int any_cand = 0;
};
void launch_track_gather(const BatchDev& bd, const PackRaw& raw_out, const TrackDev* tds, const TrackSel* sels, const TrackGrid& g,
                         cudaStream_t s);
void launch_scatter_rows(double* dst, const int* slot, const double* src, int n, int width, cudaStream_t s);
void launch_track_writeback(const BatchDev& bd, const TrackDev* tds, const TrackSel* sels, const TrackGrid& g, cudaStream_t s);

struct FrameDesc {
    int n_meas, n_runs;
    int meas_off;
    int run_off;
    int rs_off;
    int rounds_total;
    const double* lm_pos;
    const double* lm_weight;
    const double* cam16;
    int n_cam, pad;
    double pose7[7];
    double speed_weight, speed_dt;
    double speed_v_before[3];
    double speed_T_origin_before[7];
};
struct FrameRes {
    double pose[7];
    int n_solves, log_n, done, pad;
    SolveSummary solves[8];
};
struct MotionArgs {
    const FrameDesc* fd;
    const int* lm_slot;
    const int* cam;
    const float* u, *v, *d;
    const int* run_start;
    double* run_pw;
    unsigned char* run_active;
    unsigned char* run_rej;
    double* trim_val;
    IterRecord* log;
    FrameRes* res;
    IterRecord* res_log;
    unsigned char* res_rej;
    int log_cap, total_runs;
};
void launch_adjust_pose(const MotionArgs& a, int n_frames, const SolveParams& sp, cudaStream_t s);

cudaError_t configure_pack();
int pack_max_landmarks();
void launch_pack(const BatchDev& bd, const PackRaw& raw, cudaStream_t s);
void launch_unpack_landmarks(const BatchDev& bd, double* lm_user, unsigned char* rejected_user, cudaStream_t s);

cudaError_t configure_kernels(int nr_cap_max);
void launch_reset(const BatchDev& bd, const LaunchCfg& lc, cudaStream_t s);
int launch_pass(const BatchDev& bd, const SolveParams& sp, const LaunchCfg& lc, Counters* cnt, cudaStream_t s);
void launch_count_active(const BatchDev& bd, cudaStream_t s);
void launch_loop_cond(const BatchDev& bd, unsigned long long handle, int* pass, int max_passes, cudaStream_t s);
void launch_force_linearize(const BatchDev& bd, cudaStream_t s);
void launch_jacobian_only(const BatchDev& bd, const SolveParams& sp, cudaStream_t s);
void launch_expand_jl(const BatchDev& bd, double* out, cudaStream_t s);

}
```

limo_b200/csrc/kba_linearize.cuh:

```cuda
#pragma once
#include <type_traits>
#include "kba_device.cuh"

namespace kba {

constexpr int kLinThreads = 256;
constexpr int kLinWarps = kLinThreads / 32;

__host__ __device__ __forceinline__ int lin_tile_bound(int n_obs, int n_lm) { return n_obs / 16 + n_lm / 32 + 4; }
__device__ __forceinline__ size_t lin_tile_offset(const WinDesc& wd, int w) {
    return (size_t)(wd.obs_off / 16) + (size_t)(wd.lm_off / 32) + 4 * (size_t)w;
}

__device__ inline void build_lin_tiles(const BatchDev& bd, const WinDesc& wd, WinState& st, int w, int* s_chunk ) {
    const int* lm_ptr = bd.lm_ptr + wd.lm_off + w;
    int2* tiles = bd.lin_tile + lin_tile_offset(wd, w);
    const int per = max(64, (wd.n_lm + 511) / 512);
    const int n_chunks = (wd.n_lm + per - 1) / per;
    for (int pass = 0; pass < 2; ++pass) {
        for (int c = threadIdx.x; c < n_chunks; c += blockDim.x) {
            const int j0 = c * per, j1 = min(wd.n_lm, j0 + per);
            int n = 0, t_start = 0, t_cnt = 0;
            int2* out = tiles + (pass ? s_chunk[c] : 0);
            int o0 = lm_ptr[j0];
            for (int j = j0; j < j1; ++j) {
                const int o1 = lm_ptr[j + 1], k = o1 - o0;
                if (k > 0) {
                    const bool over = k > 32;
                    if (t_cnt > 0 && (over || t_cnt + k > 32)) { if (pass) out[n] = make_int2(t_start, t_cnt); ++n; t_cnt = 0; }
                    if (!over) { if (t_cnt == 0) t_start = o0; t_cnt += k; }
                }
                o0 = o1;
            }
            if (t_cnt > 0) { if (pass) out[n] = make_int2(t_start, t_cnt); ++n; }
            if (!pass) s_chunk[c] = n;
        }
        __syncthreads();
        if (!pass) {
            if (threadIdx.x == 0) {
                int acc = 0;
                for (int c = 0; c < n_chunks; ++c) { const int t = s_chunk[c]; s_chunk[c] = acc; acc += t; }
                if (acc > lin_tile_bound(wd.n_obs, wd.n_lm)) acc = 0;
                st.n_lin_tiles = acc;
                s_chunk[512] = acc;
            }
            __syncthreads();
            if (s_chunk[512] == 0) return;
        }
    }
}

constexpr int kLinMinBlocks = 3;
constexpr size_t kLinStaticSmem = sizeof(double) * (kFusedMaxKf * kPoseStride + kMaxCam * kCamStride + kLinWarps * 9 * 33 +
                                                    kLinWarps * 32 * 9 + kLinWarps) +
                                  sizeof(int) * (kLinWarps * 6 * 32 + kLinWarps) + sizeof(uint64_t);
static_assert(kLinStaticSmem <= 48 * 1024, "k_linearize: static shared memory over 48 KB");
template <bool kLoop>
__global__ void __launch_bounds__(kLinThreads, kLinMinBlocks) k_linearize(BatchDev bd, SolveParams sp, int n_units) {
    const int w = blockIdx.y;
    WinState& st = bd.state[w];
    if (st.phase != PH_ITERATE) return;
    const WinDesc& wd = bd.desc[w];
    const volatile WinState& vst = st;
    const auto n_tiles = [&] { return vst.n_lin_tiles; };
    const auto lin = [&] { return vst.need_linearize != 0; };
    const auto want_cost = [&] { return vst.need_linearize != 0 && vst.iter0 != 0; };
    if (wd.landmarks_fixed && !want_cost()) return;
    const int tid = threadIdx.x, lane = tid & 31, warp = tid >> 5;
    __shared__ __align__(16) double s_pose[kFusedMaxKf * kPoseStride];
    __shared__ __align__(16) double s_cam[kMaxCam * kCamStride];
    __shared__ __align__(8) uint64_t s_bar;
    __shared__ double s_cg[kLinWarps][9][33];
    __shared__ double s_ma[kLinWarps][32][9];
    __shared__ int s_ix[kLinWarps][6][32];
    __shared__ double s_red[kLinWarps];
    __shared__ int s_cnt[kLinWarps];
    for (int unit = blockIdx.x; unit < n_units; unit += gridDim.x) {
    asm volatile("" ::: "memory");
    if (unit * kLinWarps >= n_tiles()) {
        if (tid == 0 && want_cost()) bd.cost_part_x[(size_t)w * bd.cost_parts + unit] = 0.0;
        if constexpr (!kLoop) return;
        continue;
    }
    const size_t base = (size_t)wd.obs_off;
    const int* lm_ptr = bd.lm_ptr + wd.lm_off + w;
    const int t = unit * kLinWarps + warp;
    int2 tile = make_int2(0, 0);
    if (t < n_tiles()) tile = bd.lin_tile[lin_tile_offset(wd, w) + t];
    const bool have = lane < tile.y;
    const int o = tile.x + lane;
    int j = 0, kf = 0, cam = 0, row0 = -1, p0 = 0, p1 = 0;
    float mu = 0.f, mv = 0.f, md = 0.f;
    double p[3] = {0, 0, 0}, wgt = 0.0;
    bool act = false;
    if (have) {
        const size_t oo = base + o;
        j = bd.obs_lm[oo];
        kf = bd.obs_kf[oo]; cam = bd.obs_cam[oo]; row0 = bd.obs_row[oo];
        mu = bd.obs_u[oo]; mv = bd.obs_v[oo]; md = bd.obs_d[oo];
        p0 = lm_ptr[j]; p1 = lm_ptr[j + 1];
        act = bd.lm_active[wd.lm_off + j] != 0;
        const double* lmp = bd.lm[st.cur] + 3 * (size_t)(wd.lm_off + j);
        p[0] = lmp[0]; p[1] = lmp[1]; p[2] = lmp[2];
        wgt = bd.lm_weight[wd.lm_off + j];
    }
    int (*six)[32] = s_ix[warp];
    if (unit == (int)blockIdx.x) stage_window_bulk(wd, bd.rt[st.cur], bd.cam, s_pose, s_cam, &s_bar);
    six[0][lane] = kf; six[1][lane] = row0; six[2][lane] = wd.obs_off + p0; six[3][lane] = p1 - p0; six[4][lane] = wd.lm_off + j;
    six[5][lane] = have ? 1 | (act ? 2 : 0) | ((p0 - tile.x) << 2) : 0;
    double* sma = s_ma[warp][lane];
    bool ok = false;
    double hr = 0.0;
    double cg[9] = {0, 0, 0, 0, 0, 0, 0, 0, 0};
    if (act) {
        const auto evaluate = [&](auto with_cost) {
            double r[3], m[9], raw[2];
            const double br = sp.reprojection_thres * sp.reprojection_thres, bdp = sp.depth_thres * sp.depth_thres;
            ok = eval_factored<double, true, decltype(with_cost)::value>(s_pose + kPoseStride * kf, s_cam + kCamStride * cam, p,
                                                                          (double)mu, (double)mv, (double)md, wgt, br, bdp, r, m,
                                                                          sma + 6, hr, raw);
            if (!ok) return;
            {
                unsigned t;
                asm volatile("mov.u32 %0, %%tid.x;" : "=r"(t));
                s_ix[t >> 5][5][t & 31] |= 128;
            }
            gram_factored(m, sma);
            const double* R = s_pose + kPoseStride * reinterpret_cast<volatile int*>(six[0])[lane];
            double jl[9];
#pragma unroll
            for (int i = 0; i < 3; ++i) {
#pragma unroll
                for (int c = 0; c < 3; ++c) jl[3 * i + c] = m[3 * i] * R[c] + m[3 * i + 1] * R[3 + c] + m[3 * i + 2] * R[6 + c];
            }
            cg[0] = jl[0] * jl[0] + jl[3] * jl[3] + jl[6] * jl[6];
            cg[1] = jl[0] * jl[1] + jl[3] * jl[4] + jl[6] * jl[7];
            cg[2] = jl[0] * jl[2] + jl[3] * jl[5] + jl[6] * jl[8];
            cg[3] = jl[1] * jl[1] + jl[4] * jl[4] + jl[7] * jl[7];
            cg[4] = jl[1] * jl[2] + jl[4] * jl[5] + jl[7] * jl[8];
            cg[5] = jl[2] * jl[2] + jl[5] * jl[5] + jl[8] * jl[8];
#pragma unroll
// ... 137 lines not shown
```

limo_b200/csrc/kba_schur_fused.cuh:

```cuda
#pragma once

namespace kba {

constexpr int kLG = 8;
constexpr int kGC = 3 * kLG;
constexpr int kFStages = 6;
constexpr int kFMaxRs = 196;
constexpr int kFStageDoubles = kGC * kFMaxRs;
constexpr int kFObs = 128;
constexpr int kFConsumerWarps = 12;
constexpr int kFMaxKf = 32;

__constant__ unsigned char kSyrkMap12[12][7] = {
    {0xb6, 0x31, 0x61, 0x75, 0x80, 0x93, 0xaa}, {0xb1, 0x40, 0x42, 0x54, 0x84, 0x98, 0xff}, {0xb7, 0x10, 0x43, 0x52, 0x86, 0x95, 0xff},
    {0xbb, 0x32, 0x60, 0x65, 0x83, 0x99, 0xff}, {0xb9, 0x20, 0x53, 0x76, 0x94, 0xa2, 0xff}, {0xb3, 0x30, 0x62, 0x85, 0xa3, 0xa7, 0xff},
    {0xb0, 0x41, 0x66, 0x74, 0x82, 0xa9, 0xff}, {0xb8, 0x33, 0x55, 0x72, 0x81, 0x97, 0xa0}, {0xb2, 0x00, 0x44, 0x51, 0x73, 0x88, 0x96},
    {0xba, 0x11, 0x63, 0x71, 0x87, 0x90, 0xa5}, {0xb5, 0x22, 0x64, 0x70, 0x91, 0xa1, 0xa8}, {0xb4, 0x21, 0x50, 0x77, 0x92, 0xa4, 0xa6}};

__device__ __forceinline__ void mbar_arrive(uint64_t* bar) {
    asm volatile("mbarrier.arrive.shared::cta.b64 _, [%0];" ::"r"(smem_u32(bar)) : "memory");
}
__device__ __forceinline__ void cp_async_elem(double* dst, const double* src) {
    asm volatile("cp.async.ca.shared.global [%0], [%1], 8;" ::"r"(smem_u32(dst)), "l"(src) : "memory");
}
// ... 10 lines not shown
    asm volatile("cp.async.mbarrier.arrive.noinc.shared::cta.b64 [%0];" ::"r"(smem_u32(bar)) : "memory");
}
__device__ __forceinline__ void cp_async_commit() { asm volatile("cp.async.commit_group;" ::: "memory"); }
template <int N>
__device__ __forceinline__ void cp_async_wait() { asm volatile("cp.async.wait_group %0;" ::"n"(N) : "memory"); }
__device__ __forceinline__ void producer_sync() { asm volatile("bar.sync 1, 128;" ::: "memory"); }
template <int N>
__device__ __forceinline__ void reg_dec() { asm volatile("setmaxnreg.dec.sync.aligned.u32 %0;" ::"n"(N)); }
template <int N>
__device__ __forceinline__ void reg_inc() { asm volatile("setmaxnreg.inc.sync.aligned.u32 %0;" ::"n"(N)); }

constexpr size_t schur_fused_smem() {
    return (size_t)kFStages * kFStageDoubles * sizeof(double) + 24 * sizeof(uint64_t) + kFStages * kGC * sizeof(unsigned);
}
constexpr unsigned kNoRow = 0xff;
__device__ __forceinline__ unsigned dirty_rows(int a, int b, unsigned z) { return (unsigned)a | (unsigned)b << 8 | z << 16; }

#ifdef KBA_PROF
#define KBA_PROF_DECL long long pt_ = clock64(), pacc_[3] = {0, 0, 0}
#define KBA_PROF_T0 pt_ = clock64()
#define KBA_PROF_ACC(i) do { const long long n_ = clock64(); pacc_[i] += n_ - pt_; pt_ = n_; } while (0)
#define KBA_PROF_FLUSH(base) do { if (lane == 0 && bd.prof) for (int i_ = 0; i_ < 3; ++i_) atomicAdd(bd.prof + (base) + i_, (unsigned long long)pacc_[i_]); } while (0)
#else
#define KBA_PROF_DECL
#define KBA_PROF_T0
#define KBA_PROF_ACC(i)
#define KBA_PROF_FLUSH(base)
#endif

__device__ __forceinline__ void schur_split(int n_groups, int p_split, int& per, int& used) {
    per = max(8, (n_groups + p_split - 1) / p_split);
    used = max(1, min(p_split, (n_groups + per - 1) / per));
}

__device__ __forceinline__ void dmma16k4(double (&c)[4], double a0, double a1, double b0) {
    asm volatile("mma.sync.aligned.m16n8k4.row.col.f64.f64.f64.f64 {%0,%1,%2,%3}, {%4,%5}, {%6}, {%0,%1,%2,%3};\n"
                 : "+d"(c[0]), "+d"(c[1]), "+d"(c[2]), "+d"(c[3])
                 : "d"(a0), "d"(a1), "d"(b0));
}
__device__ __forceinline__ void dmma16k8(double (&c)[4], double a0, double a1, double a2, double a3, double b0, double b1) {
    asm volatile("mma.sync.aligned.m16n8k8.row.col.f64.f64.f64.f64 {%0,%1,%2,%3}, {%4,%5,%6,%7}, {%8,%9}, {%0,%1,%2,%3};\n"
                 : "+d"(c[0]), "+d"(c[1]), "+d"(c[2]), "+d"(c[3])
                 : "d"(a0), "d"(a1), "d"(a2), "d"(a3), "d"(b0), "d"(b1));
}

template <bool kL, bool kR, bool kRhs, bool kK8>
__device__ __forceinline__ void syrk_block(double (&c)[2][4], const double* pa, const double* pb, bool odd) {
    if (kK8 && !kRhs) {
#pragma unroll
        for (int kk = 0; kk < kGC; kk += 8) {
            const double* qa = pa + kk * kFMaxRs;
            const double* qb = pb + kk * kFMaxRs;
            const double a0 = qa[0], a1 = qa[8], a2 = qa[4 * kFMaxRs], a3 = qa[4 * kFMaxRs + 8];
            if (kL) dmma16k8(c[0], a0, a1, a2, a3, qb[0], qb[4 * kFMaxRs]);
            if (kR) dmma16k8(c[1], a0, a1, a2, a3, qb[8], qb[4 * kFMaxRs + 8]);
        }
    } else {
#pragma unroll
        for (int kk = 0; kk < kGC; kk += 4) {
            double a0, a1;
            if (kRhs) {
                const double a = pa[kk * kFMaxRs];
                a0 = odd ? 0.0 : a;
                a1 = odd ? a : 0.0;
            } else {
                a0 = pa[kk * kFMaxRs];
                a1 = pa[kk * kFMaxRs + 8];
            }
            if (kL) dmma16k4(c[0], a0, a1, pb[kk * kFMaxRs]);
            if (kR) dmma16k4(c[1], a0, a1, pb[kk * kFMaxRs + 8]);
        }
    }
}

template <bool kRhs, bool kK8>
__device__ __forceinline__ void syrk_halves(double (&c)[2][4], const double* pa, const double* pb, bool odd, bool lo, bool hi) {
    if (lo && hi) syrk_block<true, true, kRhs, kK8>(c, pa, pb, odd);
    else if (lo) syrk_block<true, false, kRhs, kK8>(c, pa, pb, odd);
    else if (hi) syrk_block<false, true, kRhs, kK8>(c, pa, pb, odd);
}

template <int kSlots>
__global__ void __launch_bounds__(512, 1) k_schur_fused(BatchDev bd) {
    const int w = blockIdx.y;
    const WinState& st = bd.state[w];
    if (st.phase != PH_ITERATE || st.solve_failed) return;
    const WinDesc& wd = bd.desc[w];
    if (wd.landmarks_fixed) return;
    extern __shared__ __align__(128) unsigned char fsm[];
    double* stage = reinterpret_cast<double*>(fsm);
    uint64_t* full = reinterpret_cast<uint64_t*>(fsm + (size_t)kFStages * kFStageDoubles * sizeof(double));
    uint64_t* empty = full + kFStages;
    unsigned* dirty = reinterpret_cast<unsigned*>(full + 24);
    const int tid = threadIdx.x, warp = tid >> 5, lane = tid & 31;
    const int n_f = st.n_f, nt = (n_f + 8) >> 3, trhs = n_f >> 3;
    int per, used;
    schur_split(wd.n_groups, (int)gridDim.x, per, used);
    if ((int)blockIdx.x >= used) return;
    const int g0 = blockIdx.x * per, g1 = min(wd.n_groups, g0 + per);
    const int* grs = bd.grp_rs + wd.grp_off;
    const int* gt0 = bd.grp_t0 + wd.grp_off;
    const int* gt1 = bd.grp_t1 + wd.grp_off;
    const int* gtl = bd.grp_tiles + wd.grp_off;
    if (tid == 0) {
        for (int i = 0; i < kFStages; ++i) { mbar_init(&full[i], 1); mbar_init(&empty[i], kFConsumerWarps); }
        asm volatile("fence.proxy.async.shared::cta;" ::: "memory");
    }
    for (int i = tid; i < kFStages * kGC; i += blockDim.x) dirty[i] = dirty_rows(0, kFMaxRs / 2, kNoRow);
    __syncthreads();
    auto next_group = [&](int g) { while (g < g1 && grs[g] == 0) ++g; return g; };

    if (warp >= kFConsumerWarps) {
        reg_dec<56>();

        const int pw = warp - kFConsumerWarps;
        const int* lm_ptr = bd.lm_ptr + wd.lm_off + w;
        const size_t base = (size_t)wd.obs_off, TG = (size_t)bd.tot_gp;
        const bool sync_path = wd.n_gp > 0 || wd.max_rank > 0;
        const int cj = lane / 3, cc = lane - 3 * cj;
        const int zj = lane - 24;
        int g1_ = -1, rs1 = 0, t01 = 0, t11 = 0, act1 = 0, p01 = 0, p11 = 0;
        int4 run1 = make_int4(0, 0, 0, 0);
        KBA_PROF_DECL;
        auto load_meta = [&](int g) {
            g1_ = g; act1 = 0; run1 = make_int4(0, 0, 0, 0); p01 = p11 = 0;
            if (g >= g1) return;
            rs1 = grs[g]; t01 = gt0[g]; t11 = gt1[g];
            if (lane < 24) {
                const int j = g * kLG + cj;
                if (j < wd.n_lm) { run1 = bd.lm_run[wd.lm_off + j]; p01 = lm_ptr[j]; p11 = lm_ptr[j + 1]; }
            } else {
                const int j = g * kLG + zj;
                if (j < wd.n_lm) { act1 = bd.lm_active[wd.lm_off + j]; p01 = lm_ptr[j]; p11 = lm_ptr[j + 1]; }
            }
        };
        auto nth_group = [&](int g, int n) {
            g = next_group(g);
            for (; n > 0 && g < g1; --n) g = next_group(g + 1);
            return g;
        };
        int g = nth_group(g0, pw), gi = pw;
        load_meta(g);
        while (g < g1) {
            const int rs = rs1, t0 = t01, t1 = t11, act0 = act1, p00 = p01, p10 = p11;
            const int4 run0 = run1;
            const int gnext = nth_group(g + 1, 3);
            load_meta(gnext);
            const int slot = gi % kFStages;
            KBA_PROF_T0;
            if (gi >= kFStages) mbar_wait(&empty[slot], ((gi / kFStages) - 1) & 1);
            KBA_PROF_ACC(0);
            double* sb = stage + (size_t)slot * kFStageDoubles;
            const bool no_run = lane < 24 && (run0.y < 0 || (run0.y > 0 && ((run0.z - 8 * t0) & 1)));
            const bool bulk = __ballot_sync(0xffffffffu, no_run) == 0u && !sync_path;
            if (lane < kGC) {
                unsigned* dl = dirty + slot * kGC + lane;
                const unsigned d = *dl;
                int s = 0, e = 0;
                if (bulk && run0.y > 0) { s = (run0.z - 8 * t0) >> 1; e = s + 3 * run0.y; }
                const int zl = (trhs >= t0 && trhs < t1) ? n_f - 8 * t0 : 8 * (t1 - t0) + (n_f - 8 * trhs);
                *dl = bulk ? dirty_rows(s, e, (unsigned)(zl >> 1)) : dirty_rows(0, rs >> 1, kNoRow);
                const int a = d & 0xff, b = (d >> 8) & 0xff, z = d >> 16;
                const bool zero_z = z != (int)kNoRow && (z < a || z >= b) && (z < s || z >= e);
                const int m1 = min(b, s), m2 = max(a, e);
                double2* col = reinterpret_cast<double2*>(sb + (size_t)lane * kFMaxRs);
                if (zero_z) col[z] = make_double2(0.0, 0.0);
// ... 152 lines not shown
```

Measured before the change: 1446.

## Add programmatic dependent launch and grid-stride loops to per-pass BA kernels

Adds griddepcontrol wait/trigger to most solve-pass kernels and launches them through cudaLaunchKernelEx with programmatic stream serialization, so the next kernel's launch can overlap the previous kernel's tail. PDL is on by default only when no graph is used, or when KBA_PDL is set. Pose-Hessian, trim-eval and cost-eval kernels become grid-stride loops with capped grids chosen by strided_grid, which cuts CTA count and repeated window staging per CTA. The trade-off is less parallelism when the grid is capped, plus an extra barrier per loop iteration.

```diff
diff --git a/limo_b200/csrc/kba_api.cu b/limo_b200/csrc/kba_api.cu
--- a/limo_b200/csrc/kba_api.cu
+++ b/limo_b200/csrc/kba_api.cu
@@ -115,11 +115,12 @@
         std::vector<unsigned char> key;
         Counters per_pass;
         int mode = 0, passes_per_launch = 0;
+        int pdl_edges = 0;
         bool unusable = false;
         void destroy() {
             if (exec) cudaGraphExecDestroy(exec);
             if (graph) cudaGraphDestroy(graph);
-            exec = nullptr; graph = nullptr; key.clear();
+            exec = nullptr; graph = nullptr; key.clear(); pdl_edges = 0;
         }
     } sg;
     Staged<int> loop_pass;
@@ -472,6 +473,23 @@
     k.insert(k.end(), p, p + sizeof(T));
 }
 
+static bool pdl_enabled(int gmode) {
+    const char* e = getenv("KBA_PDL");
+    if (!e) return gmode == 0;
+    return atoi(e) != 0;
+}
+
+static int programmatic_edges(cudaGraph_t graph) {
+    size_t n = 0;
+    if (cudaGraphGetEdges_v2(graph, nullptr, nullptr, nullptr, &n) != cudaSuccess) { cudaGetLastError(); return -1; }
+    std::vector<cudaGraphNode_t> from(n), to(n);
+    std::vector<cudaGraphEdgeData> data(n);
+    if (n && cudaGraphGetEdges_v2(graph, from.data(), to.data(), data.data(), &n) != cudaSuccess) { cudaGetLastError(); return -1; }
+    int c = 0;
+    for (size_t i = 0; i < n; ++i) c += data[i].type == cudaGraphDependencyTypeProgrammatic ? 1 : 0;
+    return c;
+}
+
 static bool build_solve_graph(kba_batch* b, const SolveParams& sp, const LaunchCfg& lc, int mode, int max_passes, int check_every,
                               const std::vector<unsigned char>& key) {
     kba_batch::SolveGraph& g = b->sg;
@@ -498,10 +516,11 @@
         if (e == cudaSuccess) {
             capturing = true;
             rc_pass = launch_pass(b->bd, sp, lc, &per, s);
-            launch_loop_cond(b->bd, (unsigned long long)handle, b->loop_pass.d, max_passes, s);
+            launch_loop_cond(b->bd, (unsigned long long)handle, b->loop_pass.d, max_passes, lc.pdl, s);
             cudaGraph_t body = nullptr;
             e = cudaStreamEndCapture(s, &body);
             capturing = false;
+            if (e == cudaSuccess) g.pdl_edges = programmatic_edges(np.conditional.phGraph_out[0]);
         }
         g.passes_per_launch = 0;
     } else {
@@ -513,6 +532,7 @@
             b->n_active.download(s);
             e = cudaStreamEndCapture(s, &g.graph);
             capturing = false;
+            if (e == cudaSuccess) g.pdl_edges = programmatic_edges(g.graph);
         }
         g.passes_per_launch = check_every;
     }
@@ -526,7 +546,9 @@
         cudaGetLastError();
         return false;
     }
-    if (getenv("KBA_GRAPH_VERBOSE")) fprintf(stderr, "kba: solve graph built (mode %d, %lld launches per pass)\n", mode, per.launches_total);
+    if (getenv("KBA_GRAPH_VERBOSE"))
+        fprintf(stderr, "kba: solve graph built (mode %d, %lld launches per pass, %d programmatic edges)\n", mode, per.launches_total,
+                g.pdl_edges);
     g.key = key;
     g.per_pass = per;
     g.mode = mode;
@@ -724,6 +746,9 @@
     { const char* le = std::getenv("KBA_LINEARIZE"); b->lc.lin_fused = !(le && std::atoi(le) == 0); }
     { const char* le = std::getenv("KBA_LIN_GRID"); if (le) b->lc.lin_grid = std::max(-1, std::atoi(le)); }
     { const char* le = std::getenv("KBA_BS_GRID"); if (le) b->lc.bs_grid = std::max(-1, std::atoi(le)); }
+    { const char* le = std::getenv("KBA_PH_GRID"); if (le) b->lc.ph_grid = std::max(-1, std::atoi(le)); }
+    { const char* le = std::getenv("KBA_TE_GRID"); if (le) b->lc.te_grid = std::max(-1, std::atoi(le)); }
+    { const char* le = std::getenv("KBA_EC_GRID"); if (le) b->lc.ec_grid = std::max(-1, std::atoi(le)); }
     {
         auto knob = [](const char* name, int dflt) { const char* e = std::getenv(name); return e ? std::atoi(e) : dflt; };
         bd.eval_tiles_jac = std::max(1, knob("KBA_EVAL_TILES_JAC", 8));
@@ -1004,6 +1029,7 @@
     if (h->kernel_timing || launch_check_enabled() || s == nullptr || b->sg.unusable) gmode = 0;
     const bool lockstep = b->bd.sharded != 0;
     if (lockstep) gmode = (gmode && shard_graph_enabled() && b->solves_done > 0) ? 1 : 0;
+    lc.pdl = pdl_enabled(gmode);
     if (gmode) {
         std::vector<unsigned char> key;
         key.reserve(sizeof(BatchDev) + sizeof(SolveParams) + 64);
@@ -1011,6 +1037,7 @@
         key_append(key, lc.nr_cap_max); key_append(key, lc.max_rank); key_append(key, (int)lc.small_syrk); key_append(key, (int)lc.lin_fused);
         key_append(key, lc.fused_slots); key_append(key, lc.xchg.user);
         key_append(key, lc.lin_grid); key_append(key, lc.bs_grid);
+        key_append(key, lc.ph_grid); key_append(key, lc.te_grid); key_append(key, lc.ec_grid); key_append(key, (int)lc.pdl);
         if (!(b->sg.exec && b->sg.key == key) && !build_solve_graph(b, sp, lc, gmode, max_passes, check_every, key)) gmode = 0;
     }
     if (gmode == 2) {
diff --git a/limo_b200/csrc/kba_device.cuh b/limo_b200/csrc/kba_device.cuh
--- a/limo_b200/csrc/kba_device.cuh
+++ b/limo_b200/csrc/kba_device.cuh
@@ -10,6 +10,9 @@
 constexpr int kCamStride = 16;
 constexpr int kIterLogCap = 160;
 constexpr int kFusedMaxKf = 32;
+
+__device__ __forceinline__ void pdl_wait() { asm volatile("griddepcontrol.wait;" ::: "memory"); }
+__device__ __forceinline__ void pdl_trigger() { asm volatile("griddepcontrol.launch_dependents;" ::: "memory"); }
 
 struct WinDesc {
     int n_kf, n_cam, n_lm, n_obs, n_gp;
diff --git a/limo_b200/csrc/kba_kernels.cu b/limo_b200/csrc/kba_kernels.cu
--- a/limo_b200/csrc/kba_kernels.cu
+++ b/limo_b200/csrc/kba_kernels.cu
@@ -15,6 +15,8 @@
 
 constexpr int kBeginThreads = 1024;
 __global__ void __launch_bounds__(kBeginThreads) k_solve_begin(BatchDev bd, SolveParams sp) {
+    pdl_wait();
+    pdl_trigger();
     const int w = blockIdx.x;
     WinState& st = bd.state[w];
     if (st.phase != PH_SOLVE_BEGIN) return;
@@ -187,7 +189,9 @@
 }
 
 template <bool kJac, int kMinBlocks, typename TLin, bool kJl = true, bool kCs = false>
-__global__ void __launch_bounds__(256, kMinBlocks) k_eval_obs(BatchDev bd, SolveParams sp, int tiles) {
+__global__ void __launch_bounds__(256, kMinBlocks) k_eval_obs(BatchDev bd, SolveParams sp, int tiles, int n_units) {
+    pdl_wait();
+    pdl_trigger();
     const int w = blockIdx.y;
     WinState& st = bd.state[w];
     const WinDesc& wd = bd.desc[w];
@@ -205,7 +209,10 @@
     __shared__ float s_cam_f[kF32 ? kMaxCam * kCamStride : 1];
     const int buf = kJac ? st.cur : 1 - st.cur;
     const double* __restrict__ lm_buf = bd.lm[buf];
-    const int i0 = blockIdx.x * tiles * 256 + threadIdx.x;
+    const int unit_end = kJac ? blockIdx.x + 1 : n_units;
+#pragma unroll 1
+    for (int unit = blockIdx.x; unit < unit_end; unit += gridDim.x) {
+    const int i0 = unit * tiles * 256 + threadIdx.x;
     int idx_b = (i0 < n_obs) ? bd.obs_lm[(size_t)obs_off + i0] : -1;
     int idx_a = (tiles > 1 && i0 + 256 < n_obs) ? bd.obs_lm[(size_t)obs_off + i0 + 256] : -1;
     int L = -1, kfi = 0, cami = 0, row = -1;
@@ -222,11 +229,13 @@
         wgt = bd.lm_weight[L];
         act = bd.lm_active[L];
     }
-    stage_window_bulk(wd, bd.rt[buf], bd.cam, s_pose, s_cam, &s_bar);
-    if (kF32) {
-        for (int i = threadIdx.x; i < wd.n_kf * kPoseStride; i += blockDim.x) s_pose_f[i] = (float)s_pose[i];
-        for (int i = threadIdx.x; i < wd.n_cam * kCamStride; i += blockDim.x) s_cam_f[i] = (float)s_cam[i];
-        __syncthreads();
+    if (unit == blockIdx.x) {
+        stage_window_bulk(wd, bd.rt[buf], bd.cam, s_pose, s_cam, &s_bar);
+        if (kF32) {
+            for (int i = threadIdx.x; i < wd.n_kf * kPoseStride; i += blockDim.x) s_pose_f[i] = (float)s_pose[i];
+            for (int i = threadIdx.x; i < wd.n_cam * kCamStride; i += blockDim.x) s_cam_f[i] = (float)s_cam[i];
+            __syncthreads();
+        }
     }
     double cost = 0.0;
     int done = 0;
@@ -300,7 +309,7 @@
         double s = 0.0;
         if (threadIdx.x == 0)
             for (int q = 0; q < 8; ++q) s += s_red[q];
-        const int slot = blockIdx.x * tiles + threadIdx.x;
+        const int slot = unit * tiles + threadIdx.x;
         if (slot < bd.cost_parts) (kJac ? bd.cost_part_x : bd.cost_part_c)[(size_t)w * bd.cost_parts + slot] = s;
     }
     if (kJac && threadIdx.x == 0) {
@@ -308,38 +317,61 @@
         for (int q = 0; q < 8; ++q) cnt += s_cnt[q];
         if (cnt) atomicAdd(bd.jac_obs, (unsigned long long)cnt);
     }
-}
+    __syncthreads();
+    }
+}
+
+template <typename... KArgs, typename... Args>
+static void launch_k(bool pdl, void (*kernel)(KArgs...), dim3 grid, dim3 block, size_t smem, cudaStream_t s, Args... args) {
+    cudaLaunchAttribute attr[1];
+    attr[0].id = cudaLaunchAttributeProgrammaticStreamSerialization;
+    attr[0].val.programmaticStreamSerializationAllowed = 1;
+    cudaLaunchConfig_t cfg = {};
+    cfg.gridDim = grid; cfg.blockDim = block; cfg.dynamicSmemBytes = smem; cfg.stream = s;
+    cfg.attrs = attr; cfg.numAttrs = pdl ? 1 : 0;
+    cudaLaunchKernelEx(&cfg, kernel, args...);
+}
+
+static int strided_grid(int cfg, int n_units, int num, int den, int n_win, int sm_count, int ctas_per_sm, int waves);
 
 template <bool kJac>
-static void launch_eval_obs(const BatchDev& bd, const SolveParams& sp, cudaStream_t s) {
+static void launch_eval_obs(const BatchDev& bd, const SolveParams& sp, cudaStream_t s, bool pdl = false, int grid_cfg = 0,
+                            int sm_count = 132) {
     const int tiles = kJac ? bd.eval_tiles_jac : bd.eval_tiles_cost;
-    const dim3 g((bd.max_obs + 256 * tiles - 1) / (256 * tiles), bd.n_win);
-    if (!kJac) { k_eval_obs<false, 4, double><<<g, 256, 0, s>>>(bd, sp, tiles); return; }
+    const int n_units = (bd.max_obs + 256 * tiles - 1) / (256 * tiles);
+    const dim3 g(n_units, bd.n_win);
+    if (!kJac) {
+        const dim3 gc(strided_grid(grid_cfg, n_units, 1, 2, bd.n_win, sm_count, 4, 4), bd.n_win);
+        launch_k(pdl, k_eval_obs<false, 4, double>, gc, dim3(256), 0, s, bd, sp, tiles, n_units);
+        return;
+    }
     const int mb = bd.eval_min_blocks;
     if (bd.precision == 1) {
-        if (bd.fused) k_eval_obs<true, 2, float, false><<<g, 256, 0, s>>>(bd, sp, tiles);
-        else k_eval_obs<true, 2, float, true><<<g, 256, 0, s>>>(bd, sp, tiles);
+        if (bd.fused) k_eval_obs<true, 2, float, false><<<g, 256, 0, s>>>(bd, sp, tiles, n_units);
+        else k_eval_obs<true, 2, float, true><<<g, 256, 0, s>>>(bd, sp, tiles, n_units);
         LCHK("k_eval_obs");
     } else if (!bd.fused) {
-        if (mb == 2) k_eval_obs<true, 2, double, true><<<g, 256, 0, s>>>(bd, sp, tiles);
-        else if (mb == 3) k_eval_obs<true, 3, double, true><<<g, 256, 0, s>>>(bd, sp, tiles);
-        else k_eval_obs<true, 4, double, true><<<g, 256, 0, s>>>(bd, sp, tiles);
+        if (mb == 2) k_eval_obs<true, 2, double, true><<<g, 256, 0, s>>>(bd, sp, tiles, n_units);
+        else if (mb == 3) k_eval_obs<true, 3, double, true><<<g, 256, 0, s>>>(bd, sp, tiles, n_units);
+        else k_eval_obs<true, 4, double, true><<<g, 256, 0, s>>>(bd, sp, tiles, n_units);
         LCHK("k_eval_obs");
     } else if (bd.eval_cs) {
-        if (mb == 2) k_eval_obs<true, 2, double, false, true><<<g, 256, 0, s>>>(bd, sp, tiles);
-        else if (mb == 3) k_eval_obs<true, 3, double, false, true><<<g, 256, 0, s>>>(bd, sp, tiles);
-        else k_eval_obs<true, 4, double, false, true><<<g, 256, 0, s>>>(bd, sp, tiles);
+        if (mb == 2) k_eval_obs<true, 2, double, false, true><<<g, 256, 0, s>>>(bd, sp, tiles, n_units);
+        else if (mb == 3) k_eval_obs<true, 3, double, false, true><<<g, 256, 0, s>>>(bd, sp, tiles, n_units);
+        else k_eval_obs<true, 4, double, false, true><<<g, 256, 0, s>>>(bd, sp, tiles, n_units);
         LCHK("k_eval_obs");
     } else {
-        if (mb == 2) k_eval_obs<true, 2, double, false><<<g, 256, 0, s>>>(bd, sp, tiles);
-        else if (mb == 3) k_eval_obs<true, 3, double, false><<<g, 256, 0, s>>>(bd, sp, tiles);
-        else k_eval_obs<true, 4, double, false><<<g, 256, 0, s>>>(bd, sp, tiles);
+        if (mb == 2) k_eval_obs<true, 2, double, false><<<g, 256, 0, s>>>(bd, sp, tiles, n_units);
+        else if (mb == 3) k_eval_obs<true, 3, double, false><<<g, 256, 0, s>>>(bd, sp, tiles, n_units);
+        else k_eval_obs<true, 4, double, false><<<g, 256, 0, s>>>(bd, sp, tiles, n_units);
         LCHK("k_eval_obs");
     }
 }
 
 template <bool kJac>
 __global__ void __launch_bounds__(256) k_gp_eval(BatchDev bd, SolveParams sp) {
+    pdl_wait();
+    pdl_trigger();
     const int w = blockIdx.x;
     const WinState& st = bd.state[w];
     if (st.phase != PH_ITERATE) return;
@@ -403,11 +435,15 @@
 template __global__ void k_gp_eval<false>(BatchDev, SolveParams);
 
 __global__ void __launch_bounds__(256, 2) k_pose_hessian(BatchDev bd, SolveParams sp) {
-    const int w = blockIdx.y, k = blockIdx.x;
+    pdl_wait();
+    pdl_trigger();
+    const int w = blockIdx.y;
     const WinState& st = bd.state[w];
     if (st.phase != PH_ITERATE || !st.need_linearize) return;
     const WinDesc& wd = bd.desc[w];
-    if (k >= wd.n_kf || bd.off_pose[wd.kf_off + k] < 0) return;
+#pragma unroll 1
+    for (int k = blockIdx.x; k < wd.n_kf; k += gridDim.x) {
+    if (bd.off_pose[wd.kf_off + k] < 0) continue;
     __shared__ double s_pose[kPoseStride];
     __shared__ double s_cam[kMaxCam * kCamStride];
     __shared__ double s_red[8][27];
@@ -508,6 +544,8 @@
         double s = 0.0;
         for (int q = 0; q < 8; ++q) s += s_red[q][threadIdx.x];
         bd.bkf[(size_t)(wd.kf_off + k) * 27 + threadIdx.x] = s;
+    }
+    __syncthreads();
     }
 }
 
@@ -825,6 +863,8 @@
 #endif
 
 __global__ void __launch_bounds__(256) k_sred_reduce(BatchDev bd, int mode) {
+    pdl_wait();
+    pdl_trigger();
     const int w = blockIdx.y;
     const WinState& st = bd.state[w];
     if (st.phase != PH_ITERATE || st.solve_failed) return;
@@ -864,6 +904,8 @@
 
 template <bool kTiled>
 __global__ void __launch_bounds__(512, 1) k_reduced_solve(BatchDev bd, SolveParams sp, int stage) {
+    pdl_wait();
+    pdl_trigger();
     const int w = blockIdx.x;
     WinState& st = bd.state[w];
     if (st.phase != PH_ITERATE) return;
@@ -1548,6 +1590,8 @@
 
 template <bool kLoop>
 __global__ void __launch_bounds__(256) k_backsub_v(BatchDev bd, int n_units) {
+    pdl_wait();
+    pdl_trigger();
     const int w = blockIdx.y;
     const WinState& st = bd.state[w];
     if (st.phase != PH_ITERATE) return;
@@ -1688,6 +1732,8 @@
 }
 
 __global__ void __launch_bounds__(128) k_lm_update(BatchDev bd, SolveParams sp) {
+    pdl_wait();
+    pdl_trigger();
     const int w = (blockIdx.x * blockDim.x + threadIdx.x) >> 5, lane = threadIdx.x & 31;
     if (w >= bd.n_win) return;
     WinState& st = bd.state[w];
@@ -1732,7 +1778,9 @@
     });
 }
 
-__global__ void __launch_bounds__(256) k_trim_eval(BatchDev bd, SolveParams sp) {
+__global__ void __launch_bounds__(256) k_trim_eval(BatchDev bd, SolveParams sp, int n_units) {
+    pdl_wait();
+    pdl_trigger();
     const int w = blockIdx.y;
     const WinState& st = bd.state[w];
     if (st.phase != PH_TRIM) return;
@@ -1742,8 +1790,10 @@
     stage_window(wd, bd.pose[st.cur], bd.cam, s_pose, s_cam);
     __syncthreads();
     const int lane = threadIdx.x & 31;
+#pragma unroll 1
+    for (int unit = blockIdx.x; unit < n_units; unit += gridDim.x)
     for (int it = 0; it < 8; ++it) {
-    const int j = (blockIdx.x * 8 + it) * 8 + (threadIdx.x >> 5);
+    const int j = (unit * 8 + it) * 8 + (threadIdx.x >> 5);
     if (j >= wd.n_lm) continue;
     const int L = wd.lm_off + j;
     double m_d = -1.0, m_r = -1.0;
@@ -1785,6 +1835,8 @@
 }
 
 __global__ void __launch_bounds__(512) k_trim_select(BatchDev bd, SolveParams sp) {
+    pdl_wait();
+    pdl_trigger();
     const int w = blockIdx.x;
     WinState& st = bd.state[w];
     if (st.phase != PH_TRIM) return;
@@ -1923,30 +1975,32 @@
 int launch_pass(const BatchDev& bd, const SolveParams& sp, const LaunchCfg& lc, Counters* cnt, cudaStream_t s) {
     const int B = bd.n_win;
     const dim3 g_obs((bd.max_obs + 255) / 256, B);
-    const dim3 g_lm((bd.max_lm + 63) / 64, B);
+    const int n_lm_units = (bd.max_lm + 63) / 64;
+    const dim3 g_lm(strided_grid(lc.te_grid, n_lm_units, 1, 8, B, lc.sm_count, 8, 1), B);
+    const dim3 g_ph(strided_grid(lc.ph_grid, bd.max_kf, 1, 3, B, lc.sm_count, 2, 8), B);
+    const bool P = lc.pdl && !bd.sharded;
     if (!bd.fused) k_panel_zero<<<dim3(64, B), 256, 0, s>>>(bd);
     LCHK("k_panel_zero");
-    k_solve_begin<<<B, kBeginThreads, 0, s>>>(bd, sp); LCHK("k_solve_begin");
+    launch_k(P, k_solve_begin, dim3(B), dim3(kBeginThreads), 0, s, bd, sp); LCHK("k_solve_begin");
     const bool timed = lc.time_jacobian && lc.ev_pool && *lc.ev_used + 2 <= lc.ev_cap;
     const bool lin1 = bd.lin1 != 0;
     if (lin1) {
-        if (bd.tot_gp > 0) k_gp_eval<true><<<B, 256, 0, s>>>(bd, sp);
+        if (bd.tot_gp > 0) launch_k(P, k_gp_eval<true>, dim3(B), dim3(256), 0, s, bd, sp);
         LCHK("k_gp_eval");
         if (timed) cudaEventRecord(lc.ev_pool[(*lc.ev_used)++], s);
         const int n_units = (lin_tile_bound(bd.max_obs, bd.max_lm) + kLinWarps - 1) / kLinWarps;
         const dim3 g_lin(strided_grid(lc.lin_grid, n_units, 1, 8, B, lc.sm_count, kLinMinBlocks, 6), B);
-        if ((int)g_lin.x < n_units) k_linearize<true><<<g_lin, kLinThreads, 0, s>>>(bd, sp, n_units);
-        else k_linearize<false><<<g_lin, kLinThreads, 0, s>>>(bd, sp, n_units);
+        launch_k(P, (int)g_lin.x < n_units ? k_linearize<true> : k_linearize<false>, g_lin, dim3(kLinThreads), 0, s, bd, sp, n_units);
         LCHK("k_linearize");
         if (timed) cudaEventRecord(lc.ev_pool[(*lc.ev_used)++], s);
-        k_pose_hessian<<<dim3(bd.max_kf, B), 256, 0, s>>>(bd, sp); LCHK("k_pose_hessian");
+        launch_k(P, k_pose_hessian, g_ph, dim3(256), 0, s, bd, sp); LCHK("k_pose_hessian");
     } else {
         if (timed) cudaEventRecord(lc.ev_pool[(*lc.ev_used)++], s);
         launch_eval_obs<true>(bd, sp, s);
         if (timed) cudaEventRecord(lc.ev_pool[(*lc.ev_used)++], s);
-        if (bd.tot_gp > 0) k_gp_eval<true><<<B, 256, 0, s>>>(bd, sp);
+        if (bd.tot_gp > 0) launch_k(P, k_gp_eval<true>, dim3(B), dim3(256), 0, s, bd, sp);
         LCHK("k_gp_eval");
-        k_pose_hessian<<<dim3(bd.max_kf, B), 256, 0, s>>>(bd, sp); LCHK("k_pose_hessian");
+        launch_k(P, k_pose_hessian, g_ph, dim3(256), 0, s, bd, sp); LCHK("k_pose_hessian");
     }
     if (bd.fused) {
         if (!lin1) {
@@ -1954,8 +2008,7 @@
             k_obs_v2<<<g_obs, 256, 0, s>>>(bd); LCHK("k_obs_v2");
         }
         const dim3 gf(bd.p_split, B);
-        if (lc.fused_slots == 7) k_schur_fused<7><<<gf, 512, schur_fused_smem(), s>>>(bd);
-        else k_schur_fused<6><<<gf, 512, schur_fused_smem(), s>>>(bd);
+        launch_k(P, lc.fused_slots == 7 ? k_schur_fused<7> : k_schur_fused<6>, gf, dim3(512), schur_fused_smem(), s, bd);
         LCHK("k_schur_fused");
     } else {
         k_landmark_reduce<false><<<dim3((bd.max_lm + 15) / 16, B), 256, 0, s>>>(bd, sp); LCHK("k_landmark_reduce");
@@ -1984,10 +2037,10 @@
         bc.sred = bd.x_recv; bc.bkf = bd.x_recv + n_s; bc.cost_part_x = bd.x_recv + n_s + n_b;
         k_sred_reduce<<<g_red, 256, 0, s>>>(bc, 2); LCHK("k_sred_reduce");
     } else if (bd.p_split > 1) {
-        k_sred_reduce<<<g_red, 256, 0, s>>>(bd, 0); LCHK("k_sred_reduce");
+        launch_k(P, k_sred_reduce, g_red, dim3(256), 0, s, bd, 0); LCHK("k_sred_reduce");
     }
     if (bd.solve_tiled) {
-        k_reduced_solve<true><<<B, 512, solve_tiled_smem(lc.nr_cap_max), s>>>(bc, sp, 0); LCHK("k_reduced_solve");
+        launch_k(P, k_reduced_solve<true>, dim3(B), dim3(512), solve_tiled_smem(lc.nr_cap_max), s, bc, sp, 0); LCHK("k_reduced_solve");
     } else if (!bd.solve_split) {
         k_reduced_solve<false><<<B, 512, solve_smem(lc.nr_cap_max), s>>>(bc, sp, 0); LCHK("k_reduced_solve");
     } else {
@@ -2003,25 +2056,24 @@
     if (bd.fused) {
         const int n_units = (bd.max_lm + 15) / 16;
         const int gx = strided_grid(lc.bs_grid, n_units, 1, 3, B, lc.sm_count, 2, 8);
-        if (gx < n_units) k_backsub_v<true><<<dim3(gx, B), 256, 0, s>>>(bd, n_units);
-        else k_backsub_v<false><<<dim3(n_units, B), 256, 0, s>>>(bd, n_units);
+        launch_k(false, gx < n_units ? k_backsub_v<true> : k_backsub_v<false>, dim3(gx, B), dim3(256), 0, s, bd, n_units);
     }
     else k_backsub<<<dim3((bd.max_lm + 15) / 16, B), 256, 0, s>>>(bd);
     LCHK("k_backsub");
-    launch_eval_obs<false>(bd, sp, s);
-    if (bd.tot_gp > 0) k_gp_eval<false><<<B, 256, 0, s>>>(bd, sp);
+    launch_eval_obs<false>(bd, sp, s, P, lc.ec_grid, lc.sm_count); LCHK("k_eval_obs");
+    if (bd.tot_gp > 0) launch_k(P, k_gp_eval<false>, dim3(B), dim3(256), 0, s, bd, sp);
     LCHK("k_gp_eval");
     if (bd.sharded) {
         k_shard_scalars<<<1, 256, 0, s>>>(bd); LCHK("k_shard_scalars");
         if (int rc = lc.xchg.allreduce(lc.xchg.user, bd.xs, bd.xs, 16 + bd.shard_world, 0, s)) return rc;
     }
-    k_lm_update<<<(B * 32 + 127) / 128, 128, 0, s>>>(bd, sp); LCHK("k_lm_update");
-    k_trim_eval<<<g_lm, 256, 0, s>>>(bd, sp); LCHK("k_trim_eval");
+    launch_k(P, k_lm_update, dim3((B * 32 + 127) / 128), dim3(128), 0, s, bd, sp); LCHK("k_lm_update");
+    launch_k(P, k_trim_eval, g_lm, dim3(256), 0, s, bd, sp, n_lm_units); LCHK("k_trim_eval");
     if (bd.sharded) {
         k_shard_trim_scatter<<<(bd.max_lm + 255) / 256, 256, 0, s>>>(bd); LCHK("k_shard_trim_scatter");
         if (int rc = lc.xchg.allreduce(lc.xchg.user, bd.trim_send, bd.trim_glob, 3LL * bd.lm_total, 0, s)) return rc;
     }
-    k_trim_select<<<B, 512, 0, s>>>(bd, sp); LCHK("k_trim_select");
+    launch_k(P, k_trim_select, dim3(B), dim3(512), 0, s, bd, sp); LCHK("k_trim_select");
     if (cnt) {
         const int gp = bd.tot_gp > 0 ? 1 : 0;
         const int prep = lin1 ? 1 : 2 + (bd.fused ? 1 : lc.max_rank + 1 + gp);
@@ -2039,6 +2091,7 @@
 }
 
 __global__ void __launch_bounds__(256) k_loop_cond(BatchDev bd, cudaGraphConditionalHandle handle, int* pass, int max_passes) {
+    pdl_wait();
     int active = 0;
     for (int w = threadIdx.x; w < bd.n_win; w += blockDim.x) active += (bd.state[w].phase != PH_DONE) ? 1 : 0;
     active = __syncthreads_count(active > 0);
@@ -2049,8 +2102,8 @@
         cudaGraphSetConditional(handle, (active > 0 && p < max_passes) ? 1u : 0u);
     }
 }
-void launch_loop_cond(const BatchDev& bd, unsigned long long handle, int* pass, int max_passes, cudaStream_t s) {
-    k_loop_cond<<<1, 256, 0, s>>>(bd, (cudaGraphConditionalHandle)handle, pass, max_passes);
+void launch_loop_cond(const BatchDev& bd, unsigned long long handle, int* pass, int max_passes, bool pdl, cudaStream_t s) {
+    launch_k(pdl && !bd.sharded, k_loop_cond, dim3(1), dim3(256), 0, s, bd, (cudaGraphConditionalHandle)handle, pass, max_passes);
 }
 
 __global__ void k_force_linearize(BatchDev bd) {
diff --git a/limo_b200/csrc/kba_kernels.h b/limo_b200/csrc/kba_kernels.h
--- a/limo_b200/csrc/kba_kernels.h
+++ b/limo_b200/csrc/kba_kernels.h
@@ -37,6 +37,10 @@
     bool lin_fused = true;
     int lin_grid = -1;
     int bs_grid = -1;
+    int ph_grid = -1;
+    int te_grid = -1;
+    int ec_grid = -1;
+    bool pdl = false;
     int fused_slots = 6;
     int rounds_override = -1, min_landmarks_for_trimming = 100, num_rounds_option = 1;
     bool time_jacobian = false;
@@ -139,7 +143,7 @@
 void launch_reset(const BatchDev& bd, const LaunchCfg& lc, cudaStream_t s);
 int launch_pass(const BatchDev& bd, const SolveParams& sp, const LaunchCfg& lc, Counters* cnt, cudaStream_t s);
 void launch_count_active(const BatchDev& bd, cudaStream_t s);
-void launch_loop_cond(const BatchDev& bd, unsigned long long handle, int* pass, int max_passes, cudaStream_t s);
+void launch_loop_cond(const BatchDev& bd, unsigned long long handle, int* pass, int max_passes, bool pdl, cudaStream_t s);
 void launch_force_linearize(const BatchDev& bd, cudaStream_t s);
 void launch_jacobian_only(const BatchDev& bd, const SolveParams& sp, cudaStream_t s);
 void launch_expand_jl(const BatchDev& bd, double* out, cudaStream_t s);
diff --git a/limo_b200/csrc/kba_linearize.cuh b/limo_b200/csrc/kba_linearize.cuh
--- a/limo_b200/csrc/kba_linearize.cuh
+++ b/limo_b200/csrc/kba_linearize.cuh
@@ -57,6 +57,8 @@
 static_assert(kLinStaticSmem <= 48 * 1024, "k_linearize: static shared memory over 48 KB");
 template <bool kLoop>
 __global__ void __launch_bounds__(kLinThreads, kLinMinBlocks) k_linearize(BatchDev bd, SolveParams sp, int n_units) {
+    pdl_wait();
+    pdl_trigger();
     const int w = blockIdx.y;
     WinState& st = bd.state[w];
     if (st.phase != PH_ITERATE) return;
diff --git a/limo_b200/csrc/kba_schur_fused.cuh b/limo_b200/csrc/kba_schur_fused.cuh
--- a/limo_b200/csrc/kba_schur_fused.cuh
+++ b/limo_b200/csrc/kba_schur_fused.cuh
@@ -116,6 +116,8 @@
 
 template <int kSlots>
 __global__ void __launch_bounds__(512, 1) k_schur_fused(BatchDev bd) {
+    pdl_wait();
+    pdl_trigger();
     const int w = blockIdx.y;
     const WinState& st = bd.state[w];
     if (st.phase != PH_ITERATE || st.solve_failed) return;
```

Result: no change. 1452 (median of 6 runs) (+0.4%).
